# intelligent-machine-learning/tfplus

Hardware: AMD Instinct MI355X
Metric: lookups+GroupAdam-applies/sec and HBM GB/s, 1M int64 ids x dim32 (higher is better)
Workload: dtype f32; 1 GPU; configs[1]: 50M-key KvVariable x dim32 per GPU, 1000000 ids/batch per GPU Zipf(1.2), lookup + sparse GroupAdam apply; keys=50000000, dim=32, batch=1000000, global_batch=1000000, parallelism=single GPU

## Files before the change

include/kvhip.h:

```cpp
#ifndef KVHIP_H_
#define KVHIP_H_

#include <stdint.h>

#ifdef __cplusplus
extern "C" {
#endif

typedef struct kv_table* kv_handle_t;
typedef void* kv_stream_t;

#define KV_OK 0
#define KV_INVALID_ARGUMENT 3
#define KV_RESOURCE_EXHAUSTED 8
#define KV_FAILED_PRECONDITION 9
#define KV_UNIMPLEMENTED 12
#define KV_INTERNAL 13

#define KV_DT_FLOAT 1
#define KV_DT_INT32 3
#define KV_DT_INT64 9
#define KV_DT_UINT64 23

#define KV_SCATTER_ASSIGN 0
// ... 30 lines not shown
                        float* out, kv_stream_t stream);
int kv_gather_or_insert_pairs(kv_handle_t h, const int64_t* id_count_pairs, int64_t n, float* out,
                              kv_stream_t stream);

typedef uint64_t kv_batch_token_t;
int kv_gather_or_insert_tok(kv_handle_t h, const void* ids, const int32_t* counts, int64_t n,
                            float* out, kv_batch_token_t* token, kv_stream_t stream);

int kv_gather_or_zeros(kv_handle_t h, const void* ids, int64_t n, float* out, kv_stream_t stream);


int kv_apply_group_adam(kv_handle_t var, kv_handle_t m_v_linear, const float* grad, const void* ids,
                        int64_t n, float lr, float beta1_power, float beta2_power, float beta1,
                        float beta2, float epsilon, float l1, float l2, float l21, int version,
                        kv_stream_t stream);
int kv_apply_adagrad(kv_handle_t var, kv_handle_t accum, float lr, const float* grad,
                     const void* ids, int64_t n, int update_slots, kv_stream_t stream);
int kv_apply_sparse_group_ftrl(kv_handle_t var, kv_handle_t accum, kv_handle_t linear,
                               const float* grad, const void* ids, int64_t n, float lr, float l1,
                               float l2, float l21, float l2_shrinkage, float lr_power,
                               kv_stream_t stream);

int kv_apply_group_adam_unique(kv_handle_t var, kv_handle_t m_v_linear, const float* grad, const void* ids, int64_t n,
                               float lr, float beta1_power, float beta2_power, float beta1, float beta2, float epsilon,
                               float l1, float l2, float l21, int version, kv_stream_t stream);
int kv_apply_adagrad_unique(kv_handle_t var, kv_handle_t accum, float lr, const float* grad, const void* ids,
                            int64_t n, int update_slots, kv_stream_t stream);
int kv_apply_sparse_group_ftrl_unique(kv_handle_t var, kv_handle_t accum, kv_handle_t linear, const float* grad,
                                      const void* ids, int64_t n, float lr, float l1, float l2, float l21,
                                      float l2_shrinkage, float lr_power, kv_stream_t stream);

int kv_apply_group_adam_tok(kv_handle_t var, kv_handle_t m_v_linear, const float* grad, const void* ids,
                            int64_t n, float lr, float beta1_power, float beta2_power, float beta1,
                            float beta2, float epsilon, float l1, float l2, float l21, int version,
                            kv_batch_token_t token, kv_stream_t stream);
int kv_apply_adagrad_tok(kv_handle_t var, kv_handle_t accum, float lr, const float* grad, const void* ids,
                         int64_t n, int update_slots, kv_batch_token_t token, kv_stream_t stream);
int kv_apply_sparse_group_ftrl_tok(kv_handle_t var, kv_handle_t accum, kv_handle_t linear, const float* grad,
                                   const void* ids, int64_t n, float lr, float l1, float l2, float l21,
                                   float l2_shrinkage, float lr_power, kv_batch_token_t token,
                                   kv_stream_t stream);

int kv_attach_slot(kv_handle_t var, kv_handle_t slot, kv_stream_t stream);

#define KV_ORDER_ARRIVAL 0
#define KV_ORDER_FIXED 1
#define KV_ORDER_OCCURRENCE 2
int kv_set_deterministic(kv_handle_t h, int on);

int kv_set_fast_math(kv_handle_t h, int on);

#define KV_STAT_MIRROR_APPLIES 0
#define KV_STAT_MIRROR_EPOCHS 1
int kv_get_stat(kv_handle_t h, int which, int64_t* value);

int kv_prepare_capture(kv_handle_t h, int64_t max_new_ids, kv_stream_t stream);

int kv_dedup_segment_sum(kv_handle_t h, const void* ids, const float* grad, int64_t n,
                         int64_t* uniq_ids, float* summed, int32_t* inverse, int64_t* num_unique,
                         kv_stream_t stream);

int kv_export_count(kv_handle_t h, int first_n, int64_t* counts, kv_stream_t stream);
int kv_export_fill(kv_handle_t h, int first_n, int64_t* keys, float* values, int64_t* blacklist,
                   int64_t* freq_keys, uint32_t* freq_values, kv_stream_t stream);
int kv_set_delta_tracking(kv_handle_t h, int support_delta_export, int support_prediction_delta_export);
int kv_export_delta_count(kv_handle_t h, int first_n, int64_t* counts, kv_stream_t stream);
int kv_export_delta_fill(kv_handle_t h, int first_n, int64_t* keys, float* values, int64_t* blacklist,
                         int64_t* freq_keys, uint32_t* freq_values, int64_t* delete_keys,
                         kv_stream_t stream);
int kv_import(kv_handle_t h, const int64_t* keys, const float* values, int64_t n,
              const int64_t* blacklist, int64_t n_blacklist, const int64_t* freq_keys,
              const uint32_t* freq_values, int64_t n_freq, kv_stream_t stream);

int kv_import_delta(kv_handle_t h, const int64_t* keys, const float* values, int64_t n,
                    const int64_t* blacklist, int64_t n_blacklist, const int64_t* freq_keys,
                    const uint32_t* freq_values, int64_t n_freq, const int64_t* delete_keys,
                    int64_t n_delete, int first_n, kv_stream_t stream);

int kv_insert(kv_handle_t h, const void* ids, const float* values, int64_t n, kv_stream_t stream);
int kv_scatter_update(kv_handle_t h, const void* ids, const float* updates, int64_t n, int op,
                      kv_stream_t stream);

int kv_unique(kv_handle_t h, const void* ids, const int32_t* counts, int64_t n, int64_t* uniq,
              int32_t* uniq_counts, int32_t* inverse, int64_t* num_unique, int64_t* num_unique_dev,
              kv_stream_t stream);

int kv_get_count(kv_handle_t h, const void* ids, int64_t n, int32_t* counts, kv_stream_t stream);
int kv_get_timestamp(kv_handle_t h, const void* ids, int64_t n, uint32_t* days, kv_stream_t stream);
int kv_delete(kv_handle_t h, const void* ids, int64_t n, int64_t* num_deleted, kv_stream_t stream);
int kv_delete_with_timestamp(kv_handle_t h, int threshold, int dry_run, int64_t* delete_keys,
                             int64_t* count, kv_stream_t stream);

int kv_batch_gather_or_zeros(int num_tables, const kv_handle_t* tables, const void* const* ids,
                             const int64_t* ns, float* const* outs, kv_stream_t stream);

int kv_multi_gather_or_insert(int num_tables, const kv_handle_t* tables, const void* const* ids,
                              const int32_t* const* counts, const int64_t* ns, float* const* outs,
                              kv_stream_t stream);
int kv_multi_apply_group_adam(int num_tables, const kv_handle_t* vars, const kv_handle_t* slots,
                              const float* const* grads, const void* const* ids, const int64_t* ns,
                              float lr, float beta1_power, float beta2_power, float beta1, float beta2,
                              float epsilon, float l1, float l2, float l21, int version,
                              kv_stream_t stream);
int kv_multi_apply_adagrad(int num_tables, const kv_handle_t* vars, const kv_handle_t* accums, float lr,
                           const float* const* grads, const void* const* ids, const int64_t* ns,
                           int update_slots, kv_stream_t stream);
// ... 155 lines not shown
```

tfplus_amd/csrc/kv_apply.hip:

```cpp
#include <hip/hip_runtime.h>

#include <type_traits>

#include "kv_host.h"

using namespace kvhip_internal;

namespace {

static bool claim_slot(kv_table* v, kv_table* sl, hipStream_t s) {
  if (v->slot_uid == sl->uid && v->slot_gen == sl->gen) return true;
  if (v->slot_uid != 0 && v->slot_uid != sl->uid) return false;
  if (v->slot_uid == sl->uid)
    launch_clear_hints(v, s);
  v->slot_uid = sl->uid;
  v->slot_gen = sl->gen;
  return true;
}

static void wrap_uniq_serial(kv_table* v, hipStream_t s) {
  if (v->uniq_serial < 65535u) return;
  launch_clear_stamps(v, s);
  v->uniq_serial = 0;
}
// ... 55 lines not shown
  }
  {
    std::vector<kv_table*> u(all);
    std::sort(u.begin(), u.end());
    if (std::adjacent_find(u.begin(), u.end()) != u.end())
      return fail(KV_INVALID_ARGUMENT, "batched op: a table is listed twice (var or slot)");
  }
  const int device = vars[0]->device;
  DeviceGuard dg(device);
  hipStream_t s = (hipStream_t)stream;
  MultiLock lock(all);
  auto keep = [&](const kv_table* tb) -> unsigned {
    unsigned k = KEEP_NONE;
    if (!two_slots(OPT))
      for (int i = 0; i < num_tables; ++i) k |= (vars[i] == tb ? KEEP_VAR : KEEP_NONE) | (slots0[i] == tb ? KEEP_SLOT : KEEP_NONE);
    return k;
  };
  if (unique && fused_ok(D) && !stream_is_capturing(s)) {
    long long nmax = 0;
    if ((rc = lock.enter(s, keep))) return rc;
    for (int i = 0; i < num_tables; ++i) {
      if ((rc = ensure_capacity(vars[i], ns[i], s)) || (rc = ensure_capacity(slots0[i], ns[i], s)) ||
          (slots1 && (rc = ensure_capacity(slots1[i], ns[i], s))))
        return rc;
      nmax = std::max<long long>(nmax, ns[i]);
    }
    if (nmax == 0) return KV_OK;
    Staged<MultiDesc> hd(device, 1, num_tables);
    if (hd.rc) return hd.rc;
    for (int i = 0; i < num_tables; ++i) {
      kv_table* v = vars[i];
      wrap_uniq_serial(v, s);
      MultiDesc& d = hd[i];
      opt_part_args(d.a, v, slots0[i], slots1 ? slots1[i] : nullptr, a, grads[i], ns[i], s);
      if ((rc = mirror_decide(v, slots0[i], d.a, !two_slots(OPT), s))) return rc;
      d.a.uniq_serial = ns[i] > 0 ? ++v->uniq_serial : 0u;
      d.ids = ids[i];
      d.n = ns[i];
    }
    const MultiDesc* md;
    if ((rc = hd.upload(s, &md))) return rc;
    const int ids32 = vars[0]->key_dtype == KV_DT_INT32 ? 1 : 0;
    ProfScope ps(vars[0], KV_PROF_APPLY_UNIQUE, s);
    rc = launch_uapply<OPT>(hd[0].a, nullptr, ids32, nmax, s, md, num_tables);
    if (rc) return fail(rc, "batched unique apply: no kernel for dim %d", D);
    HIP_TRY(hipGetLastError());
    return KV_OK;
  }
  const bool fz = fused_ok(D);
  bool reuse = tokens != nullptr && fz;
  bool pa_reuse = reuse;
  for (int i = 0; i < num_tables && reuse; ++i)
    if (ns[i] > 0) {
      const bool held = tokens[i] != 0 && tokens[i] == vars[i]->batch_serial && ns[i] == vars[i]->batch_n && vars[i]->fused_index;
      if (!held) reuse = false;
      if (!held || !vars[i]->part_pending) pa_reuse = false;
    }
  if (!reuse) pa_reuse = false;
  for (kv_table* tb : lock.ts) {
    bool taken = false;
    if (pa_reuse)
      for (int i = 0; i < num_tables; ++i) taken = taken || (vars[i] == tb && ns[i] > 0);
    if ((rc = enter_op(tb, s, keep(tb), !taken))) return rc;
  }
  long long nmax = 0;
  if (require_reuse && !reuse)
    return fail(KV_FAILED_PRECONDITION, "batched sharded apply: another op used a table since this batch's lookup");
  for (int i = 0; i < num_tables; ++i) {
    if (!reuse) vars[i]->batch_serial = 0;
    if (!reuse && (rc = ensure_capacity(vars[i], ns[i], s))) return rc;
    if ((rc = ensure_capacity(slots0[i], ns[i], s))) return rc;
    if (slots1 && (rc = ensure_capacity(slots1[i], ns[i], s))) return rc;
    if ((rc = ensure_workspace(vars[i], std::max<long long>(ns[i], 1), true, s))) return rc;
    nmax = std::max<long long>(nmax, ns[i]);
  }
  if (nmax == 0) return KV_OK;
  Staged<MultiDesc> hd(device, 1, num_tables);
  if (hd.rc) return hd.rc;
  WsDev wmax{};
  for (int i = 0; i < num_tables; ++i) {
    MultiDesc& d = hd[i];
    d.w = ws_view(vars[i], std::max<long long>(ns[i], 1), selfs ? &selfs[i] : nullptr);
    if (fz) { d.a.epart = d.w.epart; use_partitions(d.w, fused_default_P(std::max<long long>(ns[i], 1))); }
    opt_part_args(d.a, vars[i], slots0[i], slots1 ? slots1[i] : nullptr, a, grads[i], ns[i], s);
    d.a.det = vars[i]->deterministic ? 1 : 0;
    if ((rc = mirror_decide(vars[i], slots0[i], d.a, fz && !two_slots(OPT), s))) return rc;
    d.ids = ids[i];
    d.n = ns[i];
    if (ns[i] == 0) d.w.ntiles = 0;
    if (reuse && ns[i] > 0 && vars[i]->index_P) use_partitions(d.w, vars[i]->index_P);
    d.a.day_lk = d.a.day;
    if (pa_reuse && ns[i] > 0) {
      PartArgs pend;
      take_pending_part(vars[i], &pend);
      d.a.day_lk = pend.day; d.a.count_once = pend.count_once;
    }
    widen(wmax, d.w);
  }
  const MultiDesc* md;
  if ((rc = hd.upload(s, &md))) return rc;
  if (fz) {
    int pa_mode = pa_reuse ? PA_LOOKUP : PA_NONE;
    if (!reuse) {
      for (int i = 0; i < num_tables; ++i) vars[i]->fused_index = true;
      launch_ltile(vars[0], hd[0].a.tv, wmax, nullptr, nullptr, nmax, nullptr, s, -1, md, num_tables, false);
      pa_mode = PA_APPLYIDX;
      for (int i = 0; i < num_tables; ++i)
        if (ns[i] > 0) { vars[i]->batch_serial = ++g_serial; vars[i]->batch_n = ns[i]; vars[i]->index_P = hd[i].w.P; }
    }
    if ((rc = launch_tsum(hd[0].a.tv, wmax, nullptr, s, md, num_tables)))
      return fail(rc, "tile sums: no kernel for dim %d", D);
    rc = launch_papply<OPT>(wmax, hd[0].a, pa_mode, s, md, num_tables);
    if (rc) return fail(rc, "partition + apply pass: no kernel for dim %d", D);
    HIP_TRY(hipGetLastError());
    return KV_OK;
  }
  for (int i = 0; i < num_tables; ++i) vars[i]->fused_index = false;
  launch_tile<false>(vars[0], wmax, nullptr, nullptr, nmax, s, -1, md, num_tables, wmax.ntiles);
  launch_part_keys<MODE_APPLYIDX>(wmax, hd[0].a, s, md, num_tables);
  launch_order(hd[0].a.tv, wmax, nmax, s, md, num_tables);
  if ((rc = launch_apply<MODE_APPLY, OPT>(vars[0], wmax, hd[0].a, nmax, s, md, num_tables))) return rc;
  HIP_TRY(hipGetLastError());
  return KV_OK;
}

template <int OPT>
static int apply_common(kv_table* v, kv_table* s0, kv_table* s1, const float* grad, const void* ids, int64_t n,
                        const OptArgs& a, kv_batch_token_t token, hipStream_t s, bool unique, const SelfSegment* self) {
  const long long nmax = fused_tab(v) ? FUSED_MAX_N : (1ll << 21);
  if (n < 0 || n > nmax)
    return fail(n < 0 ? KV_INVALID_ARGUMENT : KV_UNIMPLEMENTED,
                "indices: %lld ids in one optimizer call (limit %lld for this embedding dim; split the batch)", (long long)n, nmax);
  if (n > 0 && (!grad || !ids)) return fail(KV_INVALID_ARGUMENT, "grad / indices pointer is null");
  if (!dim_supported(v->dim))
    return fail(KV_UNIMPLEMENTED, "embedding dim %d not supported by the fused kernels", v->dim);
  int rc;
  if (unique && fused_ok(v->dim) && !stream_is_capturing(s)) {
    if ((rc = ensure_capacity(v, n, s)) || (rc = ensure_capacity(s0, n, s)) || (s1 && (rc = ensure_capacity(s1, n, s)))) return rc;
    wrap_uniq_serial(v, s);
    PartArgs pa{};
    opt_part_args(pa, v, s0, s1, a, grad, n, s);
    if ((rc = mirror_decide(v, s0, pa, !two_slots(OPT), s))) return rc;
    pa.uniq_serial = ++v->uniq_serial;
    ProfScope ps(v, KV_PROF_APPLY_UNIQUE, s);
    rc = launch_uapply<OPT>(pa, ids, v->key_dtype == KV_DT_INT32 ? 1 : 0, n, s);
    if (rc) return fail(rc, "unique apply: no kernel for dim %d", v->dim);
    HIP_TRY(hipGetLastError());
    return KV_OK;
  }
  const bool reuse = token != 0 && token == v->batch_serial && n == v->batch_n;
  const bool pa_route = fused_tab(v);
  int pa_mode = -1;
  PartArgs pend{};
  const void* tile_ids = nullptr;
  if (v->part_pending) {
    if (reuse && pa_route && v->fused_index) {
      take_pending_part(v, &pend);
      pa_mode = PA_LOOKUP;
    } else if ((rc = flush_part(v, s))) {
      return rc;
    }
  }
  if (!reuse && (rc = ensure_capacity(v, n, s))) return rc;
  if ((rc = ensure_capacity(s0, n, s))) return rc;
  if (s1 && (rc = ensure_capacity(s1, n, s))) return rc;
  if ((rc = ensure_workspace(v, n, true, s))) return rc;
  WsDev wd = ws_view(v, n, self);
  PartArgs pa{};
  opt_part_args(pa, v, s0, s1, a, grad, n, s);
  pa.det = det_mode(v);
  pa.day_lk = pa.day;
  if (pa_mode == PA_LOOKUP) { pa.day_lk = pend.day; pa.count_once = pend.count_once; }
  if (!reuse) {
    v->batch_serial = 0;
    if (pa_route) {
      v->fused_index = true;
      choose_partitions(v, wd, n);
      tile_ids = ids;
      pa_mode = PA_APPLYIDX;
    } else {
      index_pass<MODE_APPLYIDX>(v, wd, pa, ids, nullptr, n, -1, nullptr, s);
    }
    v->batch_serial = ++g_serial;
    v->batch_n = n;
  } else if (pa_mode < 0 && v->fused_index) {
    pa_mode = PA_NONE;
  }
  if (v->fused_index && reuse && v->index_P) use_partitions(wd, v->index_P);
  if ((rc = mirror_decide(v, s0, pa, v->fused_index && !two_slots(OPT), s))) return rc;
  if (v->fused_index) rc = fused_apply<OPT>(v, wd, pa, n, s, pa_mode, tile_ids);
  else rc = launch_apply<MODE_APPLY, OPT>(v, wd, pa, n, s);
  if (rc) return rc;
  HIP_TRY(hipGetLastError());
  return KV_OK;
}


static int check_hp(float lr, float l1, float l2, float l21, float lr_power, float l2s) {
  if (!(lr > 0.f)) return fail(KV_INVALID_ARGUMENT, "lr is not a positive scalar: %g", lr);
  if (!(l1 >= 0.f)) return fail(KV_INVALID_ARGUMENT, "l1 regularization strength is not a non-negative scalar: %g", l1);
  if (!(l2 >= 0.f)) return fail(KV_INVALID_ARGUMENT, "l2 regularization strength is not a non-negative scalar: %g", l2);
  if (!(l21 >= 0.f)) return fail(KV_INVALID_ARGUMENT, "l21 regularization strength is not a non-negative scalar: %g", l21);
  if (!(lr_power <= 0.f)) return fail(KV_INVALID_ARGUMENT, "lr_power is not a non-positive scalar: %g", lr_power);
  if (!(l2s >= 0.f)) return fail(KV_INVALID_ARGUMENT, "l2 shrinkage regularization strength is not a non-negative scalar: %g", l2s);
  return KV_OK;
}

static OptCall group_adam_call(int version, float lr, float b1p, float b2p, float b1, float b2, float eps, float l1, float l2,
                               float l21) {
  OptCall c;
  if (version != 3 && version != 4) {
    c.status = fail(KV_INVALID_ARGUMENT, "GroupAdam version %d: 3 or 4", version);
    return c;
  }
  c.opt = version == 4 ? OPT_ADAM_V4 : OPT_ADAM_V3;
  c.slot_mult = 3;
  if ((c.status = check_hp(lr, l1, l2, l21, 0.f, 0.f))) return c;
  OptArgs& a = c.a;
  a.lr = lr; a.b1p = b1p; a.b2p = b2p; a.b1 = b1; a.b2 = b2; a.eps = eps;
  if (version == 4) {
    a.l1 = l1 * lr; a.l2 = l2 * lr; a.l21 = l21 * lr;
    a.alpha = lr * std::sqrt(1.f - b2p) / (1.f - b1p);
  } else {
    a.l1 = l1; a.l2 = l2; a.l21 = l21;
    a.alpha = std::sqrt(1.f - b2p) / (1.f - b1p);
  }
  return c;
}
static OptCall adagrad_call(float lr, int update_slots) {
  OptCall c;
  c.opt = OPT_ADAGRAD;
  c.a.lr = lr; c.a.update_slots = update_slots;
  return c;
}
static OptCall sparse_group_ftrl_call(float lr, float l1, float l2, float l21, float l2s, float lr_power) {
  OptCall c;
  c.opt = OPT_FTRL;
  if ((c.status = check_hp(lr, l1, l2, l21, lr_power, l2s))) return c;
  c.a.lr = lr; c.a.l1 = l1; c.a.l2 = l2; c.a.l21 = l21; c.a.l2s = l2s; c.a.lr_power = lr_power;
  return c;
}
// ... 280 lines not shown
```

tfplus_amd/csrc/kv_device.h:

```cpp
#pragma once

constexpr long long EMPTY_KEY = (long long)0x8000000000000000ULL;
constexpr unsigned FLAG_BLACK = 1u;
constexpr unsigned FLAG_UNDER = 2u;
constexpr unsigned FLAG_DIRTY = 4u;
constexpr float CUTOFF = 1.0e-20f;
constexpr unsigned FLAG_FREE = 8u;
constexpr unsigned ROW_TOMB = 0xFFFFFFFFu;
constexpr unsigned ROW_FILTERED = 0x80000000u;
constexpr unsigned ROW_MASK = 0x7FFFFFFFu;
constexpr unsigned HEAD_BIT = 0x80000000u;
constexpr unsigned BASE_MASK = 0x3FFFFFFFu;
constexpr int RANK_SHIFT = 21;
constexpr unsigned SLOT_MASK = (1u << RANK_SHIFT) - 1u;
constexpr int LCOLD = 16;
constexpr int HC = 128;
constexpr unsigned EP_TAG = 0x40000000u;
constexpr unsigned NEW_BIT = 0x80000000u;
constexpr unsigned HINT_NEW = 0xFFFFFFFFu;
constexpr int HC2 = 512;

constexpr int TB = 256;
#ifndef KV_TBT
#define KV_TBT 512
#endif
constexpr int TBT = KV_TBT;
constexpr int IPT = 4;
constexpr int TILE = TBT * IPT;
constexpr int LS = 2 * TILE;
constexpr int MAX_P = 2048;
constexpr int MAX_CHUNKS = 32768;

#ifdef KV_STAMPS
#define KV_STAMP(slot) do { if (threadIdx.x == 0) w.dbg[(size_t)blockIdx.x * 16 + (slot)] = wall_clock64(); } while (0)
#define KV_STAMPP(slot) do { if (threadIdx.x == 0) w.dbg[(size_t)(blockIdx.x + 4096) * 16 + (slot)] = wall_clock64(); } while (0)
#define KV_STAMP_HW(slot) do { if (threadIdx.x == 0) w.dbg[(size_t)blockIdx.x * 16 + (slot)] = \
    ((unsigned long long)__builtin_amdgcn_s_getreg(63508) << 32) | (unsigned)__builtin_amdgcn_s_getreg(63492); } while (0)
#define KV_STAMPPV(slot, v) do { if (threadIdx.x == 0) w.dbg[(size_t)(blockIdx.x + 4096) * 16 + (slot)] = (v); } while (0)
#define KV_STAMPA(slot) do { if (threadIdx.x == 0) w.dbg[(size_t)(blockIdx.x + 8192) * 16 + (slot)] = wall_clock64(); } while (0)
#define KV_STAMPV(slot, v) do { if (threadIdx.x == 0) w.dbg[(size_t)(blockIdx.x + 8192) * 16 + (slot)] = (v); } while (0)
#define KV_STAMPT(slot) do { if (threadIdx.x == 0) w.dbg[(size_t)(blockIdx.x + 2048) * 16 + (slot)] = wall_clock64(); } while (0)
#else
#define KV_STAMP(slot) do { } while (0)
#define KV_STAMPP(slot) do { } while (0)
#define KV_STAMP_HW(slot) do { } while (0)
#define KV_STAMPPV(slot, v) do { } while (0)
#define KV_STAMPA(slot) do { } while (0)
#define KV_STAMPV(slot, v) do { } while (0)
#define KV_STAMPT(slot) do { } while (0)
#endif

template <typename Tag, typename Kernel>
static inline int resident_blocks(Kernel k, int threads, int cap_per_cu, int fallback_per_cu) {
  constexpr int MAXDEV = 64;
  static int cache[MAXDEV];
  int dev = 0;
  hipGetDevice(&dev);
  const bool slot = dev >= 0 && dev < MAXDEV;
  if (slot) { const int c = __atomic_load_n(&cache[dev], __ATOMIC_RELAXED); if (c > 0) return c; }
  int nb = 0, cus = 0;
  hipDeviceGetAttribute(&cus, hipDeviceAttributeMultiprocessorCount, dev);
  if (hipOccupancyMaxActiveBlocksPerMultiprocessor(&nb, k, threads, 0) != hipSuccess || nb < 1) nb = fallback_per_cu;
  if (nb > cap_per_cu) nb = cap_per_cu;
  const int r = nb * (cus > 0 ? cus : 256);
  if (slot) __atomic_store_n(&cache[dev], r, __ATOMIC_RELAXED);
  return r;
}

__device__ __forceinline__ unsigned long long mix64(unsigned long long x) {
  x ^= x >> 33; x *= 0xff51afd7ed558ccdULL;
  x ^= x >> 33; x *= 0xc4ceb9fe1a85ec53ULL;
  x ^= x >> 33;
  return x;
}
__device__ __forceinline__ unsigned long long pick64(unsigned long long x) {
  x ^= x >> 30; x *= 0xbf58476d1ce4e5b9ULL;
  x ^= x >> 27; x *= 0x94d049bb133111ebULL;
  x ^= x >> 31;
  return x;
}

__device__ __forceinline__ float* row_ptr(const TableDev& t, unsigned r) {
  if (t.single || (r >> t.chunk_bits) == 0) return t.c0.rows + (size_t)r * t.dim;
// ... 599 lines not shown
```

tfplus_amd/csrc/kv_fused.h:

```cpp
#pragma once

__device__ __forceinline__ unsigned tile_insert(const TableDev& t, long long key) {
  Entry* slot;
  unsigned long long stored;
  unsigned long long p = 0;
  const bool sentinel = key == EMPTY_KEY;
  if (sentinel) { slot = &t.entries[t.mask + 1]; stored = 0ull; }
  else { stored = (unsigned long long)key; p = mix64((unsigned long long)key) & t.mask; slot = &t.entries[p]; }
  for (;;) {
    const Entry e = load_entry(slot);
    if ((unsigned long long)e.key == stored && !(sentinel && e.key == EMPTY_KEY)) {
      if (e.row == ROW_TOMB) {
        if (atomicCAS(&slot->row, ROW_TOMB, 0u) == ROW_TOMB) break;
        return NEW_BIT;
      }
      if (e.row == 0u || e.hint == HINT_NEW) return NEW_BIT | e.row;
      return e.row;
    }
    if (e.key == EMPTY_KEY) {
      const unsigned long long old = atomicCAS(reinterpret_cast<unsigned long long*>(&slot->key),
                                               (unsigned long long)EMPTY_KEY, stored);
      if (old == (unsigned long long)EMPTY_KEY) break;
      if (old == stored) return NEW_BIT;
      if (sentinel) continue;
    } else if (sentinel) {
      return NEW_BIT;
    }
    if (!sentinel) { p = (p + 1) & t.mask; slot = &t.entries[p]; }
  }
  unsigned r = 0;
  bool have = false;
  if (t.free_rows) {
    const int f = atomicSub(reinterpret_cast<int*>(&t.counters[2]), 1);
    if (f > 0) { r = t.free_rows[f - 1]; have = true; }
    else atomicAdd(reinterpret_cast<int*>(&t.counters[2]), 1);
  }
  if (!have) {
    r = atomicAdd(&t.counters[0], 1u);
    if (r >= t.max_rows) { raise_error(t, 1u); return NEW_BIT; }
  }
  *reinterpret_cast<uint2*>(&slot->row) = make_uint2(r, HINT_NEW);
  return NEW_BIT | r;
}

struct LtSmem {
  long long* lkeys;
  unsigned* lrow;
  unsigned* escan;
  unsigned* lcnt;
  unsigned short* lpos;
  unsigned* mr;
  unsigned short* lrun;
  unsigned* hist;
  unsigned* wtot;
};
constexpr size_t LT_KEYS_BYTES = (size_t)(LS + 1) * 8 + 64;
static_assert(LT_KEYS_BYTES >= (((size_t)(LS + 1) * 4 + 15) & ~(size_t)15) + (((size_t)(TILE + 1) * 4 + 15) & ~(size_t)15) + (size_t)TILE * 4, "aliases fit");

__host__ __device__ inline size_t ltile_smem_bytes() {
  size_t b = LT_KEYS_BYTES + 16;
  b += (size_t)(LS + 1) * 4 + 16;
  b += (size_t)(LS + 1) * 2 + 16;
  b += (size_t)(TILE + 1) * 2 + 16;
  b += (size_t)(MAX_P + 1) * 4 + 16;
  b += 64;
  return b;
}
__device__ __forceinline__ LtSmem carve_ltile(char* base) {
  LtSmem s;
  auto take = [&](size_t bytes) { char* p = base; base += (bytes + 15) & ~(size_t)15; return p; };
  char* k0 = take(LT_KEYS_BYTES);
  s.lkeys = reinterpret_cast<long long*>(k0);
  s.lrow = reinterpret_cast<unsigned*>(k0);
  s.escan = reinterpret_cast<unsigned*>(k0 + (((size_t)(LS + 1) * 4 + 15) & ~(size_t)15));
  s.mr = reinterpret_cast<unsigned*>(k0 + (((size_t)(LS + 1) * 4 + 15) & ~(size_t)15) + (((size_t)(TILE + 1) * 4 + 15) & ~(size_t)15));
  s.lcnt = reinterpret_cast<unsigned*>(take((size_t)(LS + 1) * 4));
  s.lpos = reinterpret_cast<unsigned short*>(take((size_t)(LS + 1) * 2));
  s.lrun = reinterpret_cast<unsigned short*>(take((size_t)(TILE + 1) * 2));
  s.hist = reinterpret_cast<unsigned*>(take((size_t)(MAX_P + 1) * 4));
  s.wtot = reinterpret_cast<unsigned*>(take(64));
  return s;
}

constexpr unsigned ES_POS = 0xFFFu, ES_NSH = 12;
static_assert(TILE <= (1 << 11), "mrow: the tile-local position is an 11-bit field");
static_assert(TILE / 2 <= (1 << 10), "mrow: the entry's epart row is a 10-bit field (an entry in mrow has >= 2 rows)");
static_assert(TILE <= (int)ES_POS && TILE / 2 < (1 << (23 - ES_NSH)), "escan: rows and entry numbers of a tile fit their fields");
static_assert(TILE <= 65535, "toff / hist / mcount pack per-tile counts into 16-bit halves");
constexpr int LT_TOUCH_MAXENT = TILE / 2;

template <typename IdT, int VQ, bool GATHER, bool NOTABLE = false>
__device__ __forceinline__ void ltile_body(const TableDev& t, const WsDev& w, const IdT* __restrict__ ids,
                                           const int* __restrict__ counts, long long n, int det,
                                           float* __restrict__ out) {
  extern __shared__ __attribute__((aligned(16))) char smem_raw[];
  LtSmem sm = carve_ltile(smem_raw);
  __shared__ unsigned lsent;

  const int tid = threadIdx.x;
  const unsigned tile = blockIdx.x;
  const long long base = (long long)tile * TILE;
  const unsigned P = w.P;
  constexpr bool PAIRS = std::is_same<IdT, IdCount>::value;
  const bool has_counts = PAIRS || counts != nullptr;
  KV_STAMP(0);
  KV_STAMP_HW(10);

  long long kreg[IPT];
  unsigned creg[IPT];
  unsigned there = 0;
#pragma unroll
  for (int k = 0; k < IPT; ++k) {
    const long long i = base + (long long)k * TBT + tid;
    if (i < n) there |= 1u << k;
    const long long ic = i < n ? i : n - 1;
    if constexpr (PAIRS) kreg[k] = load_id(((unsigned)ic - w.self_lo < w.self_len) ? static_cast<const IdT*>(w.ids_self) : ids, (size_t)ic);
    else kreg[k] = load_id(ids, (size_t)ic);
    creg[k] = 1;
  }
  if constexpr (PAIRS) {
#pragma unroll
    for (int k = 0; k < IPT; ++k) {
      const long long i = base + (long long)k * TBT + tid;
      const long long ic = i < n ? i : n - 1;
      const long long ci = (((unsigned)ic - w.self_lo < w.self_len) ? static_cast<const IdT*>(w.ids_self) : ids)[ic].count;
      creg[k] = (unsigned)(unsigned short)(ci < 65535 ? ci : 65535);
    }
  } else if (counts != nullptr) {
#pragma unroll
    for (int k = 0; k < IPT; ++k) {
      const long long i = base + (long long)k * TBT + tid;
      const int ci = counts[i < n ? i : n - 1];
      creg[k] = (unsigned)(unsigned short)(ci < 65535 ? ci : 65535);
    }
  }
  unsigned long long pp[IPT];
  Entry en[IPT];
  auto issue_probes = [&](unsigned mask) {
#pragma unroll
    for (int k = 0; k < IPT; ++k) {
      pp[k] = 0ull;
      en[k] = Entry{0, 0u, 0u};
      if constexpr (!NOTABLE) {
        pp[k] = ((mask >> k) & 1u) ? home_of(t, kreg[k], mix64((unsigned long long)kreg[k])) : 0ull;
        en[k] = load_entry(&t.entries[pp[k]]);
      }
    }
  };
  unsigned rr[IPT], hn[IPT];
  float pf = 0.f;
#pragma unroll
  for (int k = 0; k < IPT; ++k) { rr[k] = 0u; hn[k] = 0u; }
  auto resolve_probes = [&](unsigned mask) {
    if constexpr (!NOTABLE) {
#pragma unroll
      for (int k = 0; k < IPT; ++k) {
        if (!((mask >> k) & 1u)) continue;
        unsigned hint = 0;
        unsigned r = table_find_from(t, kreg[k], pp[k], en[k], &hint);
        if (__builtin_expect(r == 0u, 0)) { r = NEW_BIT; hint = 0; }
        else if (__builtin_expect(hint == HINT_NEW, 0)) { r |= NEW_BIT; hint = 0; }
        rr[k] = r; hn[k] = hint;
      }
    }
  };
  for (int s = tid; s <= LS; s += TBT) { sm.lkeys[s] = EMPTY_KEY; sm.lcnt[s] = 0; }
  for (unsigned p = tid; p <= P; p += TBT) sm.hist[p] = 0;
  if (tid == 0) lsent = 0;
  if (tile == 0 && tid == 0 && t.err_host)
    __hip_atomic_store(t.err_host + 1, w.ctr[5], __ATOMIC_RELAXED, __HIP_MEMORY_SCOPE_SYSTEM);
  lds_barrier();
  if (tile == 0 && tid < 8) w.ctr[tid] = 0;
  if constexpr (PAIRS) {
#pragma unroll
    for (int k = 0; k < IPT; ++k) {
      const long long i = base + (long long)k * TBT + tid;
      if (!((there >> k) & 1u)) continue;
      bool ok = creg[k] != 0u;
      if (ok && w.seg_cap) {
        const long long r = i % w.seg_cap;
        const long long ih = i - r;
        ok = r >= 1 && r <= (((unsigned)ih - w.self_lo < w.self_len) ? static_cast<const IdT*>(w.ids_self) : ids)[ih].id;
      }
      if (!ok) there &= ~(1u << k);
    }
  }
  lds_barrier();
  KV_STAMP(7);

  auto output_rows = [&]() {
    if constexpr (GATHER) {
      constexpr int RW = 64 / VQ;
      constexpr int CW = VQ < 8 ? VQ : 8;
      const int lane = tid & 63;
      const int v = lane % VQ, sub = lane / VQ;
      const int D4 = t.dim >> 2;
      const bool vlive = v < D4;
      const int vv = vlive ? v : 0;
      auto copy_rows = [&](auto single_tag) {
        constexpr bool SINGLE = decltype(single_tag)::value;
        const float4* rows0 = reinterpret_cast<const float4*>(t.c0.rows);
        constexpr int SPK = VQ / CW;
        constexpr int NP = IPT * SPK;
        auto issue = [&](int pc, float4 (&val)[CW]) {
          const int k = pc / SPK, j0 = (pc % SPK) * CW;
#pragma unroll
          for (int j = 0; j < CW; ++j) {
            const unsigned rj = __shfl(rr[k], (j0 + j) * RW + sub) & ROW_MASK;
            if constexpr (SINGLE) val[j] = rows0[(size_t)rj * D4 + vv];
            else val[j] = reinterpret_cast<const float4*>(row_ptr(t, rj))[vv];
          }
        };
        auto flush = [&](int pc, float4 (&val)[CW]) {
          const int k = pc / SPK, j0 = (pc % SPK) * CW;
          const long long r0 = base + (long long)k * TBT + (tid & ~63);
          if (__builtin_expect(__ballot((rr[k] & NEW_BIT) != 0u) != 0ull, 0)) {
#pragma unroll
            for (int j = 0; j < CW; ++j) {
              const unsigned rj = __shfl(rr[k], (j0 + j) * RW + sub);
              const long long kj = __shfl(kreg[k], (j0 + j) * RW + sub);
              if (rj & NEW_BIT) {
                const unsigned long long h = pick64((unsigned long long)kj ^ (t.seed * 0x9E3779B97F4A7C15ULL));
                const float4 a = reinterpret_cast<const float4*>(t.init_table + (size_t)((unsigned)h % t.init_rows) * t.dim)[vv];
                const float4 b = reinterpret_cast<const float4*>(t.init_table + (size_t)((unsigned)(h >> 32) % t.init_rows) * t.dim)[vv];
                val[j] = make_float4((a.x + b.x) * 0.5f, (a.y + b.y) * 0.5f, (a.z + b.z) * 0.5f, (a.w + b.w) * 0.5f);
// ... 29 lines not shown
          }
        } else {
#pragma unroll
          for (int pc = 0; pc < NP; ++pc) {
            issue(pc, va);
            flush(pc, va);
            asm volatile("" ::: "memory");
          }
        }
      };
      if (single_chunk(t)) copy_rows(std::true_type{}); else copy_rows(std::false_type{});
    }
  };
  unsigned tslot[IPT], myrank[IPT];
  unsigned win = 0;
#pragma unroll
  for (int k = 0; k < IPT; ++k) {
    tslot[k] = 0xFFFFFFFFu;
    myrank[k] = 0;
    if ((there >> k) & 1u) {
      const long long key = kreg[k];
      unsigned h;
      if (key == EMPTY_KEY) {
        h = LS;
        if (atomicCAS(&lsent, 0u, 1u) == 0u) win |= 1u << k;
      } else {
        h = (unsigned)(mix64((unsigned long long)key) >> 40) & (LS - 1);
        for (;;) {
          const unsigned long long old = atomicCAS(reinterpret_cast<unsigned long long*>(&sm.lkeys[h]),
                                                   (unsigned long long)EMPTY_KEY, (unsigned long long)key);
          if (old == (unsigned long long)EMPTY_KEY) { win |= 1u << k; break; }
          if (old == (unsigned long long)key) break;
          h = (h + 1) & (LS - 1);
        }
      }
      myrank[k] = atomicAdd(&sm.lcnt[h], 1u);
      tslot[k] = h;
    }
  }
  KV_STAMP(8);
  issue_probes(win);
  if constexpr (NOTABLE) {
    if (w.zero_counts) {
#pragma unroll
      for (int k = 0; k < IPT; ++k) {
        const long long i = base + (long long)k * TBT + tid;
        if (i < n) w.zero_counts[i] = 0;
      }
    }
  }
  KV_STAMP(9);
  lds_barrier();
  KV_STAMP(1);

  unsigned wcnt[IPT], wp[IPT], wr[IPT];
#pragma unroll
  for (int k = 0; k < IPT; ++k) {
    wcnt[k] = 0; wp[k] = 0; wr[k] = 0;
    if ((win >> k) & 1u) {
      wcnt[k] = sm.lcnt[tslot[k]];
      wp[k] = part_of(kreg[k], w.pshift);
      wr[k] = atomicAdd(&sm.hist[wp[k]], 1u | (wcnt[k] << 16)) & 0xFFFFu;
    }
  }
  lds_barrier();
  {
    const unsigned per = (P + TBT - 1) / TBT;
    const unsigned p0 = tid * per, p1 = min(p0 + per, P);
    unsigned sum = 0;
    for (unsigned p = p0; p < p1; ++p) sum += sm.hist[p];
    unsigned tot;
    unsigned run = block_excl_scan<TBT / 64, true>(sum, sm.wtot, &tot);
    for (unsigned p = p0; p < p1; ++p) { const unsigned c = sm.hist[p]; sm.hist[p] = run; run += c; }
    if (tid == 0) sm.hist[P] = tot;
  }
  lds_barrier();
  const unsigned nent = sm.hist[P] & 0xFFFFu;
  for (unsigned p = tid; p <= P; p += TBT) w.toff[(size_t)tile * (P + 1) + p] = sm.hist[p];
  unsigned wpos[IPT];
#pragma unroll
  for (int k = 0; k < IPT; ++k) {
    wpos[k] = 0xFFFFFFFFu;
    if ((win >> k) & 1u) {
      wpos[k] = (sm.hist[wp[k]] & 0xFFFFu) + wr[k];
      w.ent_key[(size_t)tile * TILE + wpos[k]] = kreg[k];
    }
  }
  if (det) {
    __syncthreads();
    unsigned npos[IPT];
#pragma unroll
    for (int k = 0; k < IPT; ++k) {
      npos[k] = 0xFFFFFFFFu;
      if (wpos[k] == 0xFFFFFFFFu) continue;
      const unsigned p0 = sm.hist[wp[k]] & 0xFFFFu, p1 = sm.hist[wp[k] + 1u] & 0xFFFFu;
      unsigned less = 0;
      for (unsigned j = p0; j < p1; ++j) less += w.ent_key[(size_t)tile * TILE + j] < kreg[k] ? 1u : 0u;
      npos[k] = p0 + less;
    }
    __syncthreads();
#pragma unroll
    for (int k = 0; k < IPT; ++k) {
      if (npos[k] == 0xFFFFFFFFu) continue;
      wpos[k] = npos[k];
      w.ent_key[(size_t)tile * TILE + wpos[k]] = kreg[k];
    }
  }
#pragma unroll
  for (int k = 0; k < IPT; ++k) {
    if (wpos[k] == 0xFFFFFFFFu) continue;
    sm.lpos[tslot[k]] = (unsigned short)wpos[k];
    if (!has_counts) w.ent_a[(size_t)tile * TILE + wpos[k]] = wcnt[k] | (wcnt[k] << 16);
    sm.escan[wpos[k]] = wcnt[k] > 1u ? (wcnt[k] | (1u << ES_NSH)) : 0u;
  }
  lds_barrier();
  KV_STAMP(2);

  {
    constexpr unsigned PER = (TILE + 1 + TBT - 1) / TBT;
    const unsigned e0 = tid * PER, e1 = min(e0 + PER, nent);
    unsigned sum = 0;
    for (unsigned e = e0; e < e1; ++e) sum += sm.escan[e];
    unsigned tot;
    unsigned run = block_excl_scan<TBT / 64, true>(sum, sm.wtot, &tot);
    for (unsigned e = e0; e < e1; ++e) { const unsigned c = sm.escan[e]; sm.escan[e] = run; run += c; }
    if (tid == 0) w.mcount[tile] = (tot & ES_POS) | ((tot >> ES_NSH) << 16);
  }
  resolve_probes(win);
#pragma unroll
  for (int k = 0; k < IPT; ++k) {
    if (wpos[k] == 0xFFFFFFFFu) continue;
    unsigned r = rr[k];
    if constexpr (!NOTABLE) {
      if (__builtin_expect((r & ROW_MASK) == 0u, 0)) r = tile_insert(t, kreg[k]);
    }
    const size_t e = (size_t)tile * TILE + wpos[k];
    sm.lrow[tslot[k]] = r;
    w.ent_b[e] = r;
    w.ent_base[e] = hn[k];
    if (GATHER && nent <= (unsigned)LT_TOUCH_MAXENT && (r & ROW_MASK) != 0u && !(r & NEW_BIT))
      pf += *reinterpret_cast<const volatile float*>(row_ptr(t, r & ROW_MASK));
  }
  lds_barrier();
  KV_STAMP(3);
  if (w.pos_ent) {
#pragma unroll
    for (int k = 0; k < IPT; ++k) {
      const long long i = base + (long long)k * TBT + tid;
      if (i < n) w.pos_ent[i] = tslot[k] != 0xFFFFFFFFu ? sm.lpos[tslot[k]] : (unsigned short)0xFFFFu;
    }
  }
#pragma unroll
  for (int k = 0; k < IPT; ++k) {
    if (wpos[k] == 0xFFFFFFFFu) continue;
    const unsigned pre = sm.escan[wpos[k]];
    w.ent_rec[(size_t)tile * TILE + wpos[k]] = wcnt[k] > 1u ? (EP_TAG | (tile * (unsigned)(TILE / 2) + (pre >> ES_NSH)))
                                                            : (unsigned)base + (unsigned)(k * TBT + tid);
  }
  if (det) {
    unsigned short* run = sm.lrun;
    for (int e = tid; e <= TILE; e += TBT) run[e] = 0;
    lds_barrier();
    const int lane = tid & 63, wave = tid >> 6;
#pragma unroll
    for (int k = 0; k < IPT; ++k) {
      const bool valid = tslot[k] != 0xFFFFFFFFu;
      const unsigned e = valid ? (unsigned)sm.lpos[tslot[k]] : 0u;
      unsigned long long mask = __ballot(valid);
#pragma unroll
      for (int b = 0; b < 11; ++b) {
        const bool bit = (e >> b) & 1u;
        const unsigned long long bal = __ballot(bit);
        mask &= bit ? bal : ~bal;
      }
      const unsigned rw = (unsigned)__popcll(mask & ((1ull << lane) - 1ull));
      const unsigned cnt = (unsigned)__popcll(mask);
      unsigned before = 0;
      for (int wv = 0; wv < TBT / 64; ++wv) {
        if (wave == wv && valid) {
          before = run[e];
          if (rw == 0u) run[e] = (unsigned short)(before + cnt);
        }
        lds_barrier();
      }
      myrank[k] = valid ? before + rw : 0u;
    }
  }
#pragma unroll
  for (int k = 0; k < IPT; ++k) {
    if (tslot[k] == 0xFFFFFFFFu || sm.lcnt[tslot[k]] <= 1u) continue;
    const unsigned pre = sm.escan[sm.lpos[tslot[k]]];
    sm.mr[(pre & ES_POS) + myrank[k]] = (unsigned)(k * TBT + tid) | ((pre >> ES_NSH) << 11) | (myrank[k] == 0u ? 0x80000000u : 0u);
  }
  if (has_counts) {
    lds_barrier();
    for (unsigned e = tid; e <= (unsigned)TILE; e += TBT) sm.hist[e] = 0;
    lds_barrier();
#pragma unroll
    for (int k = 0; k < IPT; ++k)
      if (tslot[k] != 0xFFFFFFFFu) atomicAdd(&sm.hist[sm.lpos[tslot[k]]], creg[k]);
    lds_barrier();
#pragma unroll
    for (int k = 0; k < IPT; ++k) {
      if (wpos[k] == 0xFFFFFFFFu) continue;
      const unsigned f = sm.hist[wpos[k]];
      w.ent_a[(size_t)tile * TILE + wpos[k]] = wcnt[k] | ((f > 65535u ? 65535u : f) << 16);
    }
  }
  lds_barrier();
  {
    unsigned* dst = w.mrow + (size_t)tile * TILE;
    for (int j = tid; j < TILE; j += TBT) dst[j] = sm.mr[j];
  }
  KV_STAMP(4);
  if constexpr (GATHER) {
#pragma unroll
    for (int k = 0; k < IPT; ++k) rr[k] = tslot[k] != 0xFFFFFFFFu ? sm.lrow[tslot[k]] : 0u;
    if (__builtin_expect(pf == 1.2345678e-38f, 0)) sm.wtot[0] = 1u;
    output_rows();
  }
  KV_STAMP(5);
}

template <typename IdT, int VQ, bool GATHER, bool NOTABLE = false>
__global__ void __launch_bounds__(TBT, 4) k_ltile(TableDev t, WsDev w, const IdT* __restrict__ ids,
                                              const int* __restrict__ counts, long long n, int det, float* __restrict__ out) {
  ltile_body<IdT, VQ, GATHER, NOTABLE>(t, w, ids, counts, n, det, out);
}

template <int T, int NW>
__device__ __forceinline__ unsigned seg_directory_t(const WsDev& w, unsigned p, unsigned short* tpre,
                                                    unsigned short* tstart, unsigned* wtot, unsigned* pbase) {
  const unsigned NT = w.ntiles;
  unsigned run0 = 0, pb = 0;
  for (unsigned tb = 0; tb < NT; tb += T) {
    const unsigned t = tb + threadIdx.x;
    unsigned len = 0, s0 = 0;
    if (t < NT) {
      const unsigned* c0 = w.toff + (size_t)t * (w.P + 1) + p;
      const unsigned a = c0[0], b = c0[1];
      s0 = a & 0xFFFFu;
      len = (b & 0xFFFFu) - s0;
      tstart[t] = (unsigned short)s0;
    }
    unsigned tot;
    const unsigned ex = block_excl_scan<NW>(len, wtot, &tot);
    unsigned tot2;
    block_excl_scan<NW>(s0, wtot, &tot2);
    if (t < NT) tpre[t] = (unsigned short)min(run0 + ex, 65535u);
    run0 += tot;
    pb += tot2;
  }
  __syncthreads();
  *pbase = pb;
  return run0;
}
__device__ __forceinline__ void part2_body(const WsDev& w, const PartArgs& a) {
  constexpr int HSK = 1024;
  constexpr int UCAPK = HSK - TBK;
  constexpr int EB = 8;
  __shared__ long long hkey[HSK + 1];
  __shared__ unsigned hval[HSK + 1];
  __shared__ unsigned hrow[HSK + 1];
  __shared__ unsigned short lnew[UCAPK + 8];
  __shared__ unsigned short ulist[UCAPK + 8];
  __shared__ unsigned lnu, lsent, lnnew, lkeys;
  __shared__ unsigned wtot[8];
  extern __shared__ __attribute__((aligned(16))) char smem_raw[];
  unsigned short* tpre = reinterpret_cast<unsigned short*>(smem_raw);
  unsigned short* tstart = tpre + w.ntiles;

  const int tid = threadIdx.x;
  const unsigned p = xcd_partition(blockIdx.x, w.P);
  const unsigned NT = w.ntiles;
  const int D = a.tv.dim;
  KV_STAMPP(0);
  unsigned pbase;
  const unsigned E = seg_directory_t<TBK, TBK / 64>(w, p, tpre, tstart, wtot, &pbase);
  if (E == 0) return;
  __shared__ unsigned stkR[24], stkr[24];
  __shared__ int sp;
  if (tid == 0) { stkR[0] = 1; stkr[0] = 0; sp = 1; lkeys = 0; }
  __syncthreads();
  if (E > 65535u) {
    if (tid == 0) raise_error(a.tv, 2u);
    return;
  }
  while (sp > 0) {
    const unsigned R = stkR[sp - 1], round = stkr[sp - 1];
    __syncthreads();
    if (tid == 0) --sp;
    for (int s = tid; s <= HSK; s += TBK) { hkey[s] = EMPTY_KEY; hval[s] = 0; hrow[s] = 0; }
    if (tid == 0) { lnu = 0; lsent = 0; lnnew = 0; }
    __syncthreads();
    for (unsigned x0 = 0; x0 < E; x0 += EB * TBK) {
      unsigned ge[EB];
      long long key[EB];
      unsigned ea[EB], rw[EB];
#pragma unroll
      for (int k = 0; k < EB; ++k) {
        const unsigned x = x0 + k * TBK + tid;
        ge[k] = x < E ? (unsigned)seg_entry(tpre, tstart, NT, x) : 0xFFFFFFFFu;
      }
#pragma unroll
      for (int k = 0; k < EB; ++k) {
        key[k] = 0; ea[k] = 0; rw[k] = 0;
        if (ge[k] != 0xFFFFFFFFu) { key[k] = w.ent_key[ge[k]]; ea[k] = w.ent_a[ge[k]]; rw[k] = w.ent_b[ge[k]]; }
      }
#pragma unroll
      for (int k = 0; k < EB; ++k) {
        if (ge[k] == 0xFFFFFFFFu || !in_round(key[k], R, round)) continue;
        if (lnu >= (unsigned)UCAPK) continue;
        bool first;
        const unsigned h = lds_key_slot<HSK>(hkey, &lsent, key[k], true, &first);
        if (first) {
          const unsigned u = atomicAdd(&lnu, 1u);
          if (u < (unsigned)UCAPK) ulist[u] = (unsigned short)h;
        }
        atomicAdd(&hval[h], ea[k] >> 16);
        atomicMax(&hrow[h], rw[k]);
      }
    }
    __syncthreads();
    if (lnu >= (unsigned)UCAPK) {
      __syncthreads();
      if (tid == 0) {
        if (sp + 2 <= 24) {
          stkR[sp] = 2 * R; stkr[sp] = round; ++sp;
          stkR[sp] = 2 * R; stkr[sp] = round + R; ++sp;
        } else {
          raise_error(a.tv, 2u);
        }
      }
      __syncthreads();
      continue;
    }
    KV_STAMPP(1);
    const unsigned nu = lnu;
    if (tid == 0) lkeys += nu;

    constexpr int PERU = (UCAPK + TBK - 1) / TBK;
    {
      unsigned sl[PERU], r[PERU];
      bool isnew[PERU];
      uint2 m[PERU];
#pragma unroll
      for (int k = 0; k < PERU; ++k) {
// ... 331 lines not shown
```

tfplus_amd/csrc/kv_host.h:

```cpp
#pragma once

#include <algorithm>
#include <atomic>
#include <cmath>
#include <cstdarg>
#include <cstdint>
#include <cstdio>
#include <cstring>
#include <mutex>
#include <string>
#include <type_traits>
#include <vector>

#include "../../include/kvhip.h"
#include "kv_launch.h"

namespace __attribute__((visibility("hidden"))) kvhip_internal {

int fail(int code, const char* fmt, ...);

#define HIP_TRY(expr)                                                                         \
  do {                                                                                        \
    hipError_t _e = (expr);                                                                   \
    if (_e != hipSuccess)                                                                     \
      return fail(_e == hipErrorOutOfMemory ? KV_RESOURCE_EXHAUSTED : KV_INTERNAL,            \
                  "%s failed: %s (%s:%d)", #expr, hipGetErrorString(_e), __FILE__, __LINE__); \
  } while (0)

struct Workspace {
  long long cap_n = 0;
  unsigned capP = 0;
  long long* ent_key = nullptr;
  unsigned* ent_a = nullptr;
  unsigned* ent_b = nullptr;
  unsigned* ent_base = nullptr;
  unsigned* ent_rec = nullptr;
  unsigned* toff = nullptr;
  unsigned* slot_rank = nullptr;
  unsigned* order = nullptr;
  uint4* coldlist = nullptr;
  uint4* hotlist = nullptr;
  uint4* litem = nullptr;
  uint4* items = nullptr;
  uint4* pmeta = nullptr;
  float* hpart = nullptr;
  long long hpart_elems = 0;
  unsigned* ctr = nullptr;
  unsigned* mcount = nullptr;
  unsigned short* pos_ent = nullptr;
  long long pos_cap = 0;
  float* epart = nullptr;
  long long epart_elems = 0;
  long long* scat_keys = nullptr;
  float* scat_sum = nullptr;
  long long scat_cap = 0;
  unsigned* seg_off = nullptr;
  long long seg_cap = 0;
  unsigned long long* dbg = nullptr;
};

}

using namespace kvhip_internal;

struct kv_table {
  uint64_t op_serial = 1, export_serial = 0, delta_serial = 0, expire_serial = 0;
  int device = 0;
  int key_dtype = KV_DT_INT64;
  int dim = 0;
  unsigned enter_threshold = 0;
  unsigned long long seed = 0;
  int fixed_day = -1;
  Entry* entries = nullptr;
  unsigned long long cap = 0;
  int chunk_bits = 16;
  std::vector<Chunk> chunks;
  Chunk* d_chunks = nullptr;
  unsigned* d_counters = nullptr;
  unsigned* free_rows = nullptr;
  unsigned long long free_cap = 0;
  long long free_known = 0;
  unsigned long long idx_ub = 0;
  unsigned long long idx_base = 0, bump_base = 1, pushes_since = 0;
  long long free_base = 0;
  unsigned long long rows_cap = 0;
  unsigned long long rows_ub = 1;
  float* init_table = nullptr;
  long long init_rows = 0;
  bool initialized = false;
  bool init_placeholder = false;
  Workspace ws;
  uint64_t batch_serial = 0;
  long long batch_n = 0;
  bool fused_index = false;
  long long batch_n_prev = 0;
  unsigned index_P = 0;
  bool part_pending = false;
  unsigned char pend_wd[sizeof(WsDev)], pend_pa[sizeof(PartArgs)];
  long long stat_mirror_applies = 0;
  std::atomic<long long> stat_mirror_epochs{0};
  TableDev mview_var{}, mview_slot{};
  kv_table* mirror_slot = nullptr;
  std::atomic<unsigned> mirror_epoch{1};
  std::atomic<bool> mirror_dirty{false};
  kv_table* mirror_var = nullptr;
  bool mirror_banned = false;
  bool mirror_shared = false;
  unsigned uniq_serial = 0;
  bool deterministic = false;
  bool occurrence_order = false;
  std::atomic<int> shard_refs{0};
  bool fast_math = false;
  uint64_t uid = 0;
  uint64_t slot_uid = 0;
  uint64_t slot_gen = 0;
  uint64_t gen = 0;
  unsigned* err_host = nullptr;
  unsigned* cnt_host = nullptr;
  hipStream_t last_stream = nullptr;
  bool has_last = false;
  hipEvent_t last_done = nullptr;
  bool track_delta = false, track_pred = false;
  std::vector<long long> del_train, del_pred;
  unsigned long long* d_stat = nullptr;
  std::mutex mu;
  unsigned* route_hist = nullptr;
  size_t route_hist_cap = 0;
  bool prof = false;
  unsigned prof_mask = 0xFFFFFFFFu;
  std::vector<hipEvent_t> ev;
  std::vector<int> ev_kind;
  size_t ev_used = 0;
  int prof_every = 1;
  unsigned prof_seq[KV_PROF_KINDS] = {};
};

namespace __attribute__((visibility("hidden"))) kvhip_internal {

inline unsigned long long pow2ceil(unsigned long long x) {
  unsigned long long p = 1;
  while (p < x) p <<= 1;
  return p;
}

inline int ilog2(unsigned long long x) {
  int l = 0;
  while ((1ull << l) < x) ++l;
  return l;
}
// ... 124 lines not shown
                  const MultiDesc* md = nullptr, int ntab = 0);
void launch_ltile(kv_table* t, const TableDev& td, const WsDev& wd, const void* ids, const int* counts, long long n, float* out,
                  hipStream_t s, int ids_kind = -1, const MultiDesc* md = nullptr, int ntab = 0, bool multi_rows = false);
void launch_part2(const WsDev& wd, const PartArgs& pa, hipStream_t s, const MultiDesc* md = nullptr, int ntab = 0);
int launch_occ_sum(const WsDev& wd, const PartArgs& pa, int fop, long long nmax, hipStream_t s);
void launch_fill_entries(kv_table* t, hipStream_t s);
void launch_clear_hints(kv_table* v, hipStream_t s);
void launch_clear_stamps(kv_table* v, hipStream_t s);
void launch_link_hints(kv_table* v, kv_table* sl, unsigned nrows, hipStream_t s);
void launch_ltile_notable(kv_table* t, const TableDev& td, const WsDev& wd, const void* ids, long long n, hipStream_t s,
                          const int* counts = nullptr, bool int32_ids = false);
void launch_ltile_multi_notable(const WsDev& wmax, int ntab, const MultiDesc* md, hipStream_t s);

enum : unsigned {
  KEEP_NONE = 0u,
  KEEP_VAR = 1u,
  KEEP_SLOT = 2u,
};

int hand_over(kv_table* t, hipStream_t s, unsigned keep = KEEP_NONE, bool settle = true, bool mutates = true);
int enter_op(kv_table* t, hipStream_t s, unsigned keep = KEEP_NONE, bool settle = true, bool mutates = true);
int join_side(kv_table* t, hipStream_t s);
int settle_pending(kv_table* t);
int stats(kv_handle_t t, hipStream_t s, unsigned long long out[2], unsigned* nrows_out);

void set_pending_part(kv_table* t, const WsDev& wd, const PartArgs& pa);
void take_pending_part(kv_table* t, PartArgs* lookup);
int flush_part(kv_table* t, hipStream_t s);
int mirror_decide(kv_table* v, kv_table* s0, PartArgs& pa, bool lean, hipStream_t s);

struct MultiLock {
  std::vector<kv_table*> ts;
  explicit MultiLock(std::initializer_list<kv_table*> l) : MultiLock(std::vector<kv_table*>(l)) {}
  explicit MultiLock(std::vector<kv_table*> l) : ts(std::move(l)) {
    std::sort(ts.begin(), ts.end());
    ts.erase(std::unique(ts.begin(), ts.end()), ts.end());
    for (auto* t : ts) t->mu.lock();
  }
  ~MultiLock() { for (auto it = ts.rbegin(); it != ts.rend(); ++it) (*it)->mu.unlock(); }
  template <class Keep>
  int enter(hipStream_t s, Keep keep, kv_table* later = nullptr) {
    int rc;
    for (auto* t : ts)
      if ((rc = enter_op(t, s, keep(t), t != later))) return rc;
    return KV_OK;
  }
  int enter(hipStream_t s) { return enter(s, [](const kv_table*) { return (unsigned)KEEP_NONE; }); }
};

void retire_stream(hipStream_t dead);

extern std::atomic<uint64_t> g_serial;
void choose_partitions(kv_table* t, WsDev& wd, long long n);
template <int MODE>
void index_pass(kv_table* t, const WsDev& wd, const PartArgs& pa, const void* ids, const int* counts, long long n,
                int ids_kind, float* out, hipStream_t s, bool file_order = true);
int fused_lookup_pass(kv_table* t, WsDev& wd, const PartArgs& pa, const void* ids, const int* counts, long long n,
                      int ids_kind, float* out, hipStream_t s, bool defer_part);
template <int MODE, int OPT>
int launch_apply(kv_table* prof_t, const WsDev& wd, const PartArgs& pa, long long nmax, hipStream_t s,
                 const MultiDesc* md = nullptr, int ntab = 0, bool skip_fin = false) {
  const int D = pa.tv.dim;
  constexpr int gmax = 2048;
  const unsigned grid = (unsigned)std::max<long long>(1, std::min<long long>(gmax, (nmax / 2 + chunk_cap(nmax)) / 4 + 1));
  const unsigned gfin = (unsigned)std::max<long long>(1, std::min<long long>(256, nmax / 4096 + 1));
  auto launch = [&](unsigned nchunks, int span) {
    if constexpr (MODE == MODE_DEDUP) return launch_dedup_fold(wd, pa, s, md, ntab, nchunks, span);
    else return launch_sorted_apply<OPT>(wd, pa, s, md, ntab, nchunks, span);
  };
  int rc;
  if (pa.det == 2 && !md) {
    const int fop = MODE == MODE_APPLY ? KV_SCATTER_ADD : pa.fold_op;
    if ((rc = launch_occ_sum(wd, pa, fop, nmax, s))) return rc;
  }
  {
    ProfScope ps(prof_t, KV_PROF_APPLY_SORTED, s);
    rc = launch(grid, 0);
  }
  if (rc == KV_OK && !skip_fin) {
    ProfScope ps(prof_t, KV_PROF_APPLY_SPAN, s);
    rc = launch(gfin, 1);
  }
  if (rc == KV_UNIMPLEMENTED)
    return md ? fail(KV_UNIMPLEMENTED, "batched launch: embedding dim %d (multiples of 4 only)", D)
              : fail(KV_UNIMPLEMENTED, "embedding dim %d not supported by the fused kernels "
                     "(multiples of 4 up to 1024, any dim up to 256)", D);
  return KV_OK;
}

struct StageSlot {
  char* host = nullptr;
  char* dev = nullptr;
  size_t cap = 0;
  hipEvent_t consumed = nullptr;
};
struct BatchStage {
  std::mutex mu;
  StageSlot slot[4];
  unsigned cursor = 0;
};
extern BatchStage g_stage[64][2];
int stage_take(BatchStage& st, size_t bytes, StageSlot** out);
template <class Desc>
class Staged {
  BatchStage& st;
  StageSlot* sl = nullptr;
  const size_t bytes;
  hipStream_t s = nullptr;
  bool launched = false;
 public:
  int rc;
// ... 47 lines not shown
```

tfplus_amd/csrc/kv_ops.hip:

```cpp
#include <hip/hip_runtime.h>

#include <iterator>

#include "kv_host.h"

using namespace kvhip_internal;

namespace {

#include "kv_device.h"
#include "kv_op_kernels.h"

static int record_deleted(kv_table* t, const void* ids, int64_t n, bool int32_ids, hipStream_t s) {
  if (!t->track_delta || n <= 0) return KV_OK;
  const size_t base = t->del_train.size();
  t->del_train.resize(base + (size_t)n);
  if (int32_ids) {
    std::vector<int> tmp((size_t)n);
    HIP_TRY(hipMemcpyAsync(tmp.data(), ids, (size_t)n * sizeof(int), hipMemcpyDeviceToHost, s));
    HIP_TRY(hipStreamSynchronize(s));
    for (int64_t i = 0; i < n; ++i) t->del_train[base + (size_t)i] = tmp[(size_t)i];
  } else {
    HIP_TRY(hipMemcpyAsync(t->del_train.data() + base, ids, (size_t)n * sizeof(long long), hipMemcpyDeviceToHost, s));
    HIP_TRY(hipStreamSynchronize(s));
// ... 97 lines not shown

static int dedup_locked(kv_table* t, const void* ids, const float* grad, int64_t n, int64_t* uniq,
                        float* summed, int32_t* inverse, int64_t* num_unique, int fold_op, hipStream_t s) {
  int rc;
  if ((rc = ensure_workspace(t, n, true, s))) return rc;
  WsDev wd = ws_view(t, n);
  t->batch_serial = 0;
  PartArgs pa = self_part_args(t, n);
  pa.grad = grad;
  pa.out_keys = (long long*)uniq;
  pa.out_sum = summed;
  pa.fold_op = fold_op;
  pa.dd_number = 1;
  if ((rc = segment_sums(t, wd, pa, ids, n, t->key_dtype == KV_DT_INT32, true, "per-id sums", s))) return rc;
  if (inverse && t->fused_index) k_inverse_e<<<nblocks(n, TB, 2048), TB, 0, s>>>(t->ws.pos_ent, wd.ent_b, n, inverse);
  else if (inverse) k_dedup_inverse<<<nblocks(n, TB, 2048), TB, 0, s>>>(wd, n, inverse);
  unsigned U = 0;
  if ((rc = read_count(t, wd.ctr, s, &U))) return rc;
  *num_unique = U;
  return KV_OK;
}

static int ensure_free_list(kv_table* t, hipStream_t s) {
  if (t->free_cap >= t->rows_cap) return KV_OK;
  unsigned* nf = nullptr;
  HIP_TRY(hipStreamSynchronize(s));
  HIP_TRY(hipMalloc(&nf, (size_t)t->rows_cap * sizeof(unsigned)));
  if (t->free_rows) {
    HIP_TRY(hipMemcpy(nf, t->free_rows, (size_t)t->free_cap * sizeof(unsigned), hipMemcpyDeviceToDevice));
    hipFree(t->free_rows);
  }
  t->free_rows = nf;
  t->free_cap = t->rows_cap;
  return KV_OK;
}

static int after_release(kv_table* t, hipStream_t s, unsigned long long* released) {
  unsigned c[3];
  unsigned long long n = 0;
  HIP_TRY(hipMemcpyAsync(&n, t->d_stat, sizeof n, hipMemcpyDeviceToHost, s));
  HIP_TRY(hipMemcpyAsync(c, t->d_counters, sizeof c, hipMemcpyDeviceToHost, s));
  HIP_TRY(hipStreamSynchronize(s));
  t->pushes_since += n;
  t->free_known = std::max(0, (int)c[2]);
  t->rows_ub = c[0];
  *released = n;
  return KV_OK;
}

static int delete_locked(kv_table* t, const void* ids, int64_t n, int64_t* num_deleted, hipStream_t s) {
  int rc;
  if ((rc = enter_op(t, s))) return rc;
  t->batch_serial = 0;
  if ((rc = ensure_free_list(t, s))) return rc;
  HIP_TRY(hipMemsetAsync(t->d_stat, 0, 4 * sizeof(unsigned long long), s));
  with_id_type(t->key_dtype == KV_DT_INT32, [&](auto id) {
    using IDT = decltype(id);
    k_delete<IDT><<<nblocks(n, TB, 4096), TB, 0, s>>>(dev_view(t), (const IDT*)ids, n, t->free_rows, t->d_stat);
  });
  HIP_TRY(hipGetLastError());
  unsigned long long rel = 0;
  if ((rc = after_release(t, s, &rel))) return rc;
  if (num_deleted) *num_deleted = (int64_t)rel;
  return KV_OK;
}

static int count_or_ts(kv_handle_t t, const void* ids, int64_t n, int what, uint32_t* out, kv_stream_t stream) {
  int rc;
  if ((rc = check_table(t))) return rc;
  if (n < 0 || (n > 0 && (!ids || !out))) return fail(KV_INVALID_ARGUMENT, "indices / output pointer is null");
  if ((rc = require_initialized(t))) return rc;
  if (n == 0) return KV_OK;
  TableOp op(t, stream);
  if ((rc = join_side(t, op.s))) return rc;
  with_id_type(t->key_dtype == KV_DT_INT32, [&](auto id) {
    using IDT = decltype(id);
    k_get_count_ts<IDT><<<nblocks(n, TB, 4096), TB, 0, op.s>>>(dev_view(t), (const IDT*)ids, n, what, today(t), out);
  });
  HIP_TRY(hipGetLastError());
  return KV_OK;
}

static int scatter_like(kv_handle_t t, const void* ids, const float* vals, int64_t n, int op,
                        int is_insert, int mark, const unsigned* fvals, hipStream_t s) {
  int rc;
  if (n == 0) return KV_OK;
  if (n < 0 || !ids || (!vals && mark < 0)) return fail(KV_INVALID_ARGUMENT, "bad arguments");
  if (!is_insert && mark < 0 && (rc = require_initialized(t))) return rc;
  const long long CH = 1ll << 21;
  const size_t idsz = t->key_dtype == KV_DT_INT32 ? 4 : 8;
  for (long long off = 0; off < n; off += CH) {
    const long long m = std::min(CH, (long long)n - off);
    if ((rc = ensure_capacity(t, m, s))) return rc;
    if ((rc = ensure_workspace(t, m, false, s))) return rc;
    const WsDev wd = ws_view(t, m);
    PartArgs pa = self_part_args(t, m);
    if (!t->initialized) {
      pa.tv.init_table = t->chunks[0].rows;
      pa.tv.init_rows = 1;
      pa.ts0 = pa.tv; pa.ts1 = pa.tv;
    }
    pa.grad = vals ? vals + (size_t)off * t->dim : nullptr;
    pa.scatter_op = op; pa.is_insert = is_insert;
    pa.mark_what = mark; pa.fvals = fvals ? fvals + off : nullptr;
    t->batch_serial = 0;
    launch_tile<true>(t, wd, (const char*)ids + (size_t)off * idsz, nullptr, m, s);
// ... 38 lines not shown
  }
  return KV_OK;
}

}

namespace __attribute__((visibility("hidden"))) kvhip_internal {
int multi_common(int num_tables, const kv_handle_t* tables, const void* const* ids, const int64_t* ns) {
  int rc;
  if ((rc = check_same_shape(num_tables, tables, "tables"))) return rc;
  if (!ids || !ns) return fail(KV_INVALID_ARGUMENT, "null argument array");
  for (int i = 0; i < num_tables; ++i) {
    if (tables[i]->dim != tables[0]->dim || tables[i]->key_dtype != tables[0]->key_dtype)
      return fail(KV_INVALID_ARGUMENT, "batched op: tables must share dim and key dtype (group them by shape)");
    if (tables[i]->occurrence_order)
      return fail(KV_UNIMPLEMENTED, "batched op: a table in occurrence-order mode (kv_set_deterministic(h, 2)) takes the per-table ops");
    if (ns[i] < 0 || ns[i] > (fused_tab(tables[0]) ? FUSED_MAX_N : (1ll << 21)))
      return fail(KV_INVALID_ARGUMENT, "indices: bad length %lld", (long long)ns[i]);
    if (ns[i] > 0 && !ids[i]) return fail(KV_INVALID_ARGUMENT, "indices pointer is null");
    if ((rc = require_initialized(tables[i]))) return rc;
    for (int j = 0; j < i; ++j)
      if (tables[j] == tables[i]) return fail(KV_INVALID_ARGUMENT, "batched op: table listed twice");
  }
  return KV_OK;
}

int gather_or_insert_impl(kv_handle_t t, const void* ids, const int32_t* counts, int64_t n, float* out,
                          kv_stream_t stream, int pairs, kv_batch_token_t* token, unsigned seg_cap,
                          const SelfSegment* self) {
  int rc;
  if ((rc = check_table(t))) return rc;
  if (n == 0) return KV_OK;
  if (n < 0 || n > (1ll << 30)) return fail(KV_INVALID_ARGUMENT, "indices: bad length %lld", (long long)n);
  if (!ids || !out) return fail(KV_INVALID_ARGUMENT, "indices / output pointer is null");
  if ((rc = require_initialized(t))) return rc;
  TableOp tab(t, stream);
  const hipStream_t s = tab.s;
  if ((rc = enter_op(t, s, KEEP_VAR))) return rc;
  const long long CHK = fused_tab(t) ? FUSED_MAX_N : (1ll << 21);
  const size_t idsz = pairs ? 16 : (t->key_dtype == KV_DT_INT32 ? 4 : 8);
  t->batch_serial = 0;
  for (long long off = 0; off < n; off += CHK) {
    const long long m = std::min(CHK, (long long)n - off);
    const void* idp = (const char*)ids + (size_t)off * idsz;
    const int32_t* cp = counts ? counts + off : nullptr;
    float* op = out + (size_t)off * t->dim;
    if ((rc = ensure_capacity(t, m, s))) return rc;
    if ((rc = ensure_workspace(t, m, false, s))) return rc;
    WsDev wd = ws_view(t, m, self);
    wd.seg_cap = seg_cap;
    PartArgs pa = self_part_args(t, m);
    pa.day = today(t);
    const bool defer_part = token != nullptr && n <= CHK;
    if (fused_tab(t)) { if ((rc = fused_lookup_pass(t, wd, pa, idp, cp, m, pairs ? 2 : -1, op, s, defer_part))) return rc; }
    else index_pass<MODE_LOOKUP>(t, wd, pa, idp, cp, m, pairs ? 2 : -1, op, s, token != nullptr && n <= CHK);
  }
  HIP_TRY(hipGetLastError());
  if (token && n <= CHK) {
    t->batch_serial = ++g_serial;
    t->batch_n = n;
    if (token) *token = t->batch_serial;
  }
  return KV_OK;
}

int multi_lookup_impl(int num_tables, const kv_handle_t* tables, const void* const* ids,
                      const int32_t* const* counts, const int64_t* ns, float* const* outs,
                      kv_batch_token_t* tokens, kv_stream_t stream, int ids_kind, const unsigned* seg_caps,
                      const SelfSegment* selfs) {
  int rc;
  if (tokens && num_tables > 0) std::memset(tokens, 0, (size_t)num_tables * sizeof(kv_batch_token_t));
  if ((rc = multi_common(num_tables, tables, ids, ns))) return rc;
  if (!outs) return fail(KV_INVALID_ARGUMENT, "null argument array");
  const int device = tables[0]->device;
  DeviceGuard dg(device);
  hipStream_t s = (hipStream_t)stream;
  MultiLock lock(std::vector<kv_table*>(tables, tables + num_tables));
  if ((rc = lock.enter(s, [](const kv_table*) { return (unsigned)KEEP_VAR; }))) return rc;
  long long nmax = 0;
  for (int i = 0; i < num_tables; ++i) {
    tables[i]->batch_serial = 0;
    if (ns[i] > 0 && !outs[i]) return fail(KV_INVALID_ARGUMENT, "output pointer is null");
    if ((rc = ensure_capacity(tables[i], ns[i], s))) return rc;
    if ((rc = ensure_workspace(tables[i], std::max<long long>(ns[i], 1), false, s))) return rc;
    nmax = std::max<long long>(nmax, ns[i]);
  }
  if (nmax == 0) return KV_OK;
  Staged<MultiDesc> hd(device, 1, num_tables);
  if (hd.rc) return hd.rc;
  WsDev wmax{};
  for (int i = 0; i < num_tables; ++i) {
    MultiDesc& d = hd[i];
    d.w = ws_view(tables[i], std::max<long long>(ns[i], 1), selfs ? &selfs[i] : nullptr);
    if (seg_caps) d.w.seg_cap = seg_caps[i];
    if (fused_tab(tables[i])) use_partitions(d.w, fused_default_P(std::max<long long>(ns[i], 1)));
    d.a = self_part_args(tables[i], ns[i]);
    d.a.day = today(tables[i]);
    d.ids = ids[i];
    d.counts = counts ? counts[i] : nullptr;
    d.out = outs[i];
    d.n = ns[i];
    if (ns[i] == 0) d.w.ntiles = 0;
    widen(wmax, d.w);
  }
  const MultiDesc* md;
  if ((rc = hd.upload(s, &md))) return rc;
  kv_table* t0 = tables[0];
  if (fused_tab(t0)) {
    for (int i = 0; i < num_tables; ++i) tables[i]->fused_index = true;
    launch_ltile(t0, hd[0].a.tv, wmax, nullptr, nullptr, nmax, nullptr, s, ids_kind, md, num_tables, true);
    const bool defer = tokens != nullptr;
    if (!defer) launch_part2(wmax, hd[0].a, s, md, num_tables);
    if (tokens)
      for (int i = 0; i < num_tables; ++i) {
        if (ns[i] <= 0) continue;
        tables[i]->batch_serial = ++g_serial;
        tables[i]->batch_n = ns[i];
        tables[i]->index_P = hd[i].w.P;
        tokens[i] = tables[i]->batch_serial;
        if (defer) set_pending_part(tables[i], hd[i].w, hd[i].a);
      }
  } else {
    for (int i = 0; i < num_tables; ++i) tables[i]->fused_index = false;
    launch_tile<false>(t0, wmax, nullptr, nullptr, nmax, s, -1, md, num_tables, wmax.ntiles);
    launch_part_keys<MODE_LOOKUP>(wmax, hd[0].a, s, md, num_tables);
    launch_gather(hd[0].a.tv, wmax, nullptr, nmax, s, md, num_tables);
  }
  HIP_TRY(hipGetLastError());
  return KV_OK;
}
}

extern "C" {

int kv_size(kv_handle_t t, int64_t* out, kv_stream_t stream) { return read_figure(t, 0, out, stream); }
int kv_sum_freq(kv_handle_t t, int64_t* out, kv_stream_t stream) { return read_figure(t, 1, out, stream); }
int kv_map_size(kv_handle_t t, int64_t* out, kv_stream_t stream) { return read_figure(t, 2, out, stream); }

int kv_get_meta(kv_handle_t t, const int64_t* ids, int64_t n, uint32_t* fw, uint8_t* fl, kv_stream_t stream) {
  int rc;
  if ((rc = check_table(t))) return rc;
  if (n <= 0) return KV_OK;
  TableOp op(t, stream);
  if ((rc = join_side(t, op.s))) return rc;
  k_get_meta<long long><<<nblocks(n, TB), TB, 0, op.s>>>(dev_view(t), (const long long*)ids, n, fw, fl);
  HIP_TRY(hipGetLastError());
  return KV_OK;
}

int kv_gather_or_insert(kv_handle_t t, const void* ids, const int32_t* counts, int64_t n, float* out,
                        kv_stream_t stream) {
  return gather_or_insert_impl(t, ids, counts, n, out, stream, 0, nullptr);
}
int kv_gather_or_insert_tok(kv_handle_t t, const void* ids, const int32_t* counts, int64_t n, float* out,
                            kv_batch_token_t* token, kv_stream_t stream) {
  if (token) *token = 0;
  return gather_or_insert_impl(t, ids, counts, n, out, stream, 0, token);
}
int kv_gather_or_insert_pairs(kv_handle_t t, const int64_t* id_count_pairs, int64_t n, float* out,
                              kv_stream_t stream) {
  if (t && t->key_dtype == KV_DT_INT32) return fail(KV_INVALID_ARGUMENT, "id/count pairs carry int64 ids");
  return gather_or_insert_impl(t, id_count_pairs, nullptr, n, out, stream, 1, nullptr);
// ... 198 lines not shown
  if (n == 0) {
    if (num_unique_dev) HIP_TRY(hipMemsetAsync(num_unique_dev, 0, sizeof(int64_t), (hipStream_t)stream));
    return KV_OK;
  }
  if (n < 0 || !ids || !uniq) return fail(KV_INVALID_ARGUMENT, "bad arguments");
  if (n > FUSED_MAX_N) return fail(KV_UNIMPLEMENTED, "%lld ids in one call (limit 2^23)", (long long)n);
  TableOp op(t, stream);
  const hipStream_t s = op.s;
  if ((rc = enter_op(t, s, KEEP_VAR | KEEP_SLOT))) return rc;
  if ((rc = ensure_workspace(t, n, false, s))) return rc;
  WsDev wd = ws_view(t, n);
  t->batch_serial = 0;
  PartArgs pa = self_part_args(t, n);
  pa.out_keys = (long long*)uniq;
  pa.out_counts = uniq_counts;
  if ((rc = fused_unique_pass(t, wd, pa, ids, counts, n, s))) return rc;
  if (inverse) k_inverse_e<<<nblocks(n, TB, 2048), TB, 0, s>>>(t->ws.pos_ent, wd.ent_b, n, inverse);
  if (num_unique_dev) k_store_count<<<1, 1, 0, s>>>(wd.ctr, (long long*)num_unique_dev);
  HIP_TRY(hipGetLastError());
  if (num_unique) {
    unsigned U = 0;
    if ((rc = read_count(t, wd.ctr, s, &U))) return rc;
    *num_unique = U;
  }
  return KV_OK;
}

int kv_delete(kv_handle_t t, const void* ids, int64_t n, int64_t* num_deleted, kv_stream_t stream) {
  int rc;
  if ((rc = check_table(t))) return rc;
  if (num_deleted) *num_deleted = 0;
  if (n < 0 || (n > 0 && !ids)) return fail(KV_INVALID_ARGUMENT, "indices pointer is null");
  if ((rc = require_initialized(t))) return rc;
  if (n == 0) return KV_OK;
  TableOp op(t, stream);
  if ((rc = record_deleted(t, ids, n, t->key_dtype == KV_DT_INT32, op.s))) return rc;
  return delete_locked(t, ids, n, num_deleted, op.s);
}

int kv_delete_with_timestamp(kv_handle_t t, int threshold, int dry_run, int64_t* out_keys, int64_t* count,
                             kv_stream_t stream) {
  int rc;
  if ((rc = check_table(t))) return rc;
  if (!count || (!dry_run && !out_keys)) return fail(KV_INVALID_ARGUMENT, "count / delete_keys pointer is null");
  if ((rc = require_initialized(t))) return rc;
  TableOp op(t, stream);
  const hipStream_t s = op.s;
  if (!dry_run) {
    if (t->expire_serial != t->op_serial)
      return fail(KV_FAILED_PRECONDITION, "the table was used between the dry run and kv_delete_with_timestamp: the key "
                                          "buffer sized from the count may be too small; count again");
    ++t->op_serial;
    t->batch_serial = 0;
  }
  unsigned nrows = 1;
  if ((rc = stats(t, s, nullptr, &nrows))) return rc;
  if (!dry_run && (rc = ensure_free_list(t, s))) return rc;
  HIP_TRY(hipMemsetAsync(t->d_stat, 0, 4 * sizeof(unsigned long long), s));
  const unsigned thr = (unsigned)(threshold & 0xFFFF);
  k_delete_by_time<<<nblocks(nrows, TB, 4096), TB, 0, s>>>(dev_view(t), nrows, today(t), thr, dry_run ? 0 : 1,
                                                        t->free_rows, t->d_stat, (long long*)out_keys);
  HIP_TRY(hipGetLastError());
  unsigned long long rel = 0;
  if (dry_run) {
    HIP_TRY(hipMemcpyAsync(&rel, t->d_stat, sizeof rel, hipMemcpyDeviceToHost, s));
    HIP_TRY(hipStreamSynchronize(s));
  } else if ((rc = after_release(t, s, &rel))) {
    return rc;
  }
  *count = (int64_t)rel;
  if (dry_run) t->expire_serial = t->op_serial;
  if (!dry_run && (rc = record_deleted(t, out_keys, (int64_t)rel, false, s))) return rc;
  return KV_OK;
}

int kv_get_count(kv_handle_t t, const void* ids, int64_t n, int32_t* counts, kv_stream_t stream) {
  return count_or_ts(t, ids, n, 0, (uint32_t*)counts, stream);
}
int kv_get_timestamp(kv_handle_t t, const void* ids, int64_t n, uint32_t* days, kv_stream_t stream) {
  return count_or_ts(t, ids, n, 1, days, stream);
}

int kv_take_rows(int device, const void* src, const int32_t* index, const int32_t* index_outer, int64_t n,
                 int64_t row_bytes, int scatter, void* out, kv_stream_t stream) {
  if (index_outer && scatter) return fail(KV_INVALID_ARGUMENT, "kv_take_rows: the two-level index is gather only");
  if (n < 0 || row_bytes <= 0 || row_bytes % 4 || (n > 0 && (!src || !index || !out)))
    return fail(KV_INVALID_ARGUMENT, "kv_take_rows: n %lld, row_bytes %lld (a positive multiple of 4)",
                (long long)n, (long long)row_bytes);
  if (n == 0) return KV_OK;
  DeviceGuard dg(device);
  hipStream_t s = (hipStream_t)stream;
  const bool wide = row_bytes % 16 == 0 && ((uintptr_t)src % 16 == 0) && ((uintptr_t)out % 16 == 0);
  const unsigned nu = (unsigned)(row_bytes / (wide ? 16 : 4));
  const int sh = (nu & (nu - 1)) == 0 ? ilog2(nu) : -1;
  const int grid = nblocks(n * nu, TB * 4, 8192);
  if (wide) {
    if (scatter) k_take_rows<float4, 1><<<grid, TB, 0, s>>>((const float4*)src, index, n, nu, sh, (float4*)out);
    else k_take_rows<float4, 0><<<grid, TB, 0, s>>>((const float4*)src, index, n, nu, sh, (float4*)out, index_outer);
  } else {
    if (scatter) k_take_rows<float, 1><<<grid, TB, 0, s>>>((const float*)src, index, n, nu, sh, (float*)out);
    else k_take_rows<float, 0><<<grid, TB, 0, s>>>((const float*)src, index, n, nu, sh, (float*)out, index_outer);
  }
  HIP_TRY(hipGetLastError());
  return KV_OK;
}

// ... 121 lines not shown
    for (long long off = 0; off < n; off += CHK) {
      const long long m = std::min(CHK, (long long)n - off);
      int64_t U = 0;
      if ((rc = dedup_locked(t, (const char*)ids + (size_t)off * idsz, updates + (size_t)off * t->dim, m,
                             (int64_t*)w.scat_keys, w.scat_sum, nullptr, &U, fold, s)))
        return rc;
      if (t->key_dtype == KV_DT_INT32 && U > 0)
        k_narrow_keys<<<1, 1024, 0, s>>>(w.scat_keys, U);
      if ((rc = scatter_like(t, w.scat_keys, w.scat_sum, U, op, 0, -1, nullptr, s))) return rc;
    }
    return KV_OK;
  }
  return scatter_like(t, ids, updates, n, op, 0, -1, nullptr, s);
}

int kv_import_delta(kv_handle_t t, const int64_t* keys, const float* values, int64_t n, const int64_t* blacklist,
                    int64_t n_black, const int64_t* fkeys, const uint32_t* fvals, int64_t n_freq,
                    const int64_t* delete_keys, int64_t n_delete, int first_n, kv_stream_t stream) {
  int rc;
  if ((rc = check_table(t))) return rc;
  TableOp op(t, stream);
  const hipStream_t s = op.s;
  if (t->key_dtype == KV_DT_INT32) return fail(KV_UNIMPLEMENTED, "import with int32 keys");
  if ((rc = enter_op(t, s))) return rc;
  if ((rc = scatter_like(t, keys, values, n, KV_SCATTER_ASSIGN, 3, -1, nullptr, s))) return rc;
  if (n_black > 0) {
    if (first_n > 3) {
      if ((rc = scatter_like(t, blacklist, nullptr, n_black, 0, 1, 0, nullptr, s))) return rc;
    } else if ((rc = delete_locked(t, blacklist, n_black, nullptr, s))) {
      return rc;
    }
  }
  if (n_freq > 0 && (rc = scatter_like(t, fkeys, nullptr, n_freq, 0, 1, 1, fvals, s))) return rc;
  if (n_delete > 0 && (rc = delete_locked(t, delete_keys, n_delete, nullptr, s))) return rc;
  if ((rc = ensure_init_placeholder(t, s))) return rc;
  t->initialized = true;
  HIP_TRY(hipGetLastError());
  return KV_OK;
}

int kv_import(kv_handle_t t, const int64_t* keys, const float* values, int64_t n, const int64_t* blacklist,
              int64_t n_black, const int64_t* fkeys, const uint32_t* fvals, int64_t n_freq,
              kv_stream_t stream) {
  int rc;
  if ((rc = check_table(t))) return rc;
  TableOp op(t, stream);
  const hipStream_t s = op.s;
  if (t->key_dtype == KV_DT_INT32) return fail(KV_UNIMPLEMENTED, "import with int32 keys");
  if ((rc = enter_op(t, s))) return rc;
  HIP_TRY(hipStreamSynchronize(s));
  t->gen += 1;
  t->slot_uid = 0;
  t->batch_serial = 0;
  unsigned init[3] = {1, 0, 0};
  HIP_TRY(hipMemcpy(t->d_counters, init, sizeof init, hipMemcpyHostToDevice));
  launch_fill_entries(t, s);
  t->rows_ub = 1;
  t->idx_ub = t->idx_base = 0; t->bump_base = 1; t->pushes_since = 0; t->free_base = 0; t->free_known = 0;
  t->del_train.clear(); t->del_pred.clear();
  if ((rc = scatter_like(t, keys, values, n, KV_SCATTER_ASSIGN, 2, -1, nullptr, s))) return rc;
  if (n_black > 0 && (rc = scatter_like(t, blacklist, nullptr, n_black, 0, 1, 0, nullptr, s))) return rc;
  if (n_freq > 0 && (rc = scatter_like(t, fkeys, nullptr, n_freq, 0, 1, 1, fvals, s))) return rc;
  if ((rc = ensure_init_placeholder(t, s))) return rc;
  t->initialized = true;
  HIP_TRY(hipGetLastError());
  return KV_OK;
}

}
```

tfplus_amd/csrc/kv_papply.h:

```cpp
#pragma once

#ifndef KV_PA_WAVES
#define KV_PA_WAVES 4
#endif
#ifndef KV_PA_HOTRB
#define KV_PA_HOTRB 8
#endif
template <int TBP> struct PaShape { static constexpr int HSK = TBP >= 512 ? 2048 : 1024, LSRC = TBP >= 512 ? 2048 : 1536; };

template <int OPT, int V, int LPR, int K, int TBP, int FM = -1>
__device__ __forceinline__ void papply_body(const WsDev& w, const PartArgs& a, const int mode_) {
  constexpr bool UQ = FM == PA_UNIQUE, DN = FM == PA_DEDUP_NUM, DD = FM == PA_DEDUP || DN;
  const int mode = FM >= 0 ? (DN ? (int)PA_DEDUP : FM) : (mode_ & 0xFF);
  constexpr int HSK = PaShape<TBP>::HSK;
  constexpr int PA_LSRC = PaShape<TBP>::LSRC;
  constexpr int UCAPK = (HSK - TBP) < 1023 ? (HSK - TBP) : 1023;
  constexpr int EB = 8;
  constexpr int G = 64 / LPR;
  constexpr int RB = (KV_PA_HOTRB / K) > 0 ? (KV_PA_HOTRB / K) : 1;
  constexpr int NW = TBP / 64;
  __shared__ long long hkey[HSK + 1];
  __shared__ unsigned hval[DD ? 1 : HSK + 1];
  __shared__ unsigned hrow[HSK + 1];
  __shared__ unsigned hhint[(UQ || DD) ? 1 : HSK + 1];
  __shared__ unsigned hocc[HSK + 1];
  __shared__ unsigned short hcn[HSK + 1];
  __shared__ unsigned short ulist[UCAPK + 8];
  __shared__ unsigned short kord[UCAPK + 8];
  __shared__ unsigned lsrc[PA_LSRC];
  __shared__ unsigned lnu, lsent, lnext, lkeys, lbase;
  __shared__ unsigned rh[MAXW], rbase[MAXW];
  __shared__ unsigned wtot[8];
  __shared__ unsigned stkR[24], stkr[24];
  __shared__ int sp;
  extern __shared__ __attribute__((aligned(16))) char smem_raw[];
  unsigned short* tpre = reinterpret_cast<unsigned short*>(smem_raw);
  unsigned short* tstart = tpre + w.ntiles;

  const int tid = threadIdx.x;
  const unsigned p = xcd_partition(blockIdx.x, w.P);
  const unsigned NT = w.ntiles;
  const int D = a.tv.dim;
  const unsigned errflag = *reinterpret_cast<volatile unsigned*>(&a.tv.counters[1]);
  KV_STAMPP(0);
  unsigned pbase = 0;
  const unsigned E = seg_directory_t<TBP, NW>(w, p, tpre, tstart, wtot, &pbase);
  KV_STAMPP(5);
  if (E == 0) return;
  if (tid == 0) { sp = 0; lkeys = 0; }
  __syncthreads();
  if (E > 65535u) {
    if (tid == 0) raise_error(a.tv, 2u);
    return;
  }
  const bool in_lds = E <= (unsigned)PA_LSRC;
  unsigned* const gsrc = w.order + pbase;
  auto src_at = [&](unsigned i) -> unsigned {
    return in_lds ? lsrc[i] : __hip_atomic_load(gsrc + i, __ATOMIC_RELAXED, __HIP_MEMORY_SCOPE_AGENT);
  };

  auto do_round = [&](const unsigned R, const unsigned round) -> bool {
    __syncthreads();
    for (int s = tid; s <= HSK; s += TBP) {
      hkey[s] = EMPTY_KEY; hrow[s] = 0; hocc[s] = 0;
      if constexpr (!DD) hval[s] = 0;
      if constexpr (!UQ && !DD) hhint[s] = 0;
    }
    if (tid == 0) { lnu = 0; lsent = 0; lnext = 0; }
    __syncthreads();
    unsigned csrc[EB];
    unsigned short cslot[EB];
    bool cin[EB];
    const bool cached = (R == 1 && E <= (unsigned)(EB * TBP));
    for (unsigned x0 = 0; x0 < E; x0 += EB * TBP) {
      unsigned ge[EB];
      long long key[EB];
      unsigned ea[EB], rw[EB], hi[EB], sr[EB];
#pragma unroll
      for (int k = 0; k < EB; ++k) {
        const unsigned x = x0 + k * TBP + tid;
        ge[k] = x < E ? (unsigned)seg_entry(tpre, tstart, NT, x) : 0xFFFFFFFFu;
      }
#pragma unroll
      for (int k = 0; k < EB; ++k) {
        key[k] = 0; ea[k] = 0; rw[k] = 0; hi[k] = 0; sr[k] = 0;
        if (ge[k] != 0xFFFFFFFFu) {
          key[k] = w.ent_key[ge[k]]; ea[k] = w.ent_a[ge[k]]; rw[k] = w.ent_b[ge[k]]; hi[k] = w.ent_base[ge[k]];
          if (cached) sr[k] = w.ent_rec[ge[k]];
        }
      }
#pragma unroll
      for (int k = 0; k < EB; ++k) {
        if (x0 == 0) { csrc[k] = sr[k]; cslot[k] = 0; cin[k] = false; }
        if (ge[k] == 0xFFFFFFFFu || !in_round(key[k], R, round)) continue;
        if (lnu >= (unsigned)UCAPK) continue;
        bool first;
        const unsigned h = lds_key_slot<HSK>(hkey, &lsent, key[k], true, &first);
        if (first) {
          const unsigned u = atomicAdd(&lnu, 1u);
          if (u < (unsigned)UCAPK) ulist[u] = (unsigned short)h;
        }
        if constexpr (UQ) atomicAdd(&hval[h], a.sparse_unique ? (ea[k] & 0xFFFFu) : (ea[k] >> 16));
        else if constexpr (!DD) { if (mode == PA_LOOKUP) atomicAdd(&hval[h], ea[k] >> 16); }
        atomicAdd(&hocc[h], 1u);
        atomicMax(&hrow[h], rw[k]);
        if constexpr (!UQ && !DD) { if (hi[k]) atomicMax(&hhint[h], hi[k]); }
        if (x0 == 0) { cslot[k] = (unsigned short)h; cin[k] = true; }
      }
    }
    __syncthreads();
    if (lnu >= (unsigned)UCAPK) return true;
    KV_STAMPP(1);
    const unsigned nu = lnu;
    const unsigned lkeys_before = lkeys;
    __syncthreads();
    if (tid == 0) {
      lkeys += nu;
      if ((UQ && !a.sparse_unique) || DN) lbase = atomicAdd(&w.ctr[0], nu);
    }

    constexpr int PERU = (UCAPK + TBP - 1) / TBP;
    unsigned nhot, ncold;
    {
      unsigned kcnt[PERU];
      unsigned sum = 0, ch = 0, hh = 0;
#pragma unroll
      for (int q = 0; q < PERU; ++q) {
        const unsigned u = tid * PERU + q;
        kcnt[q] = u < nu ? hocc[ulist[u]] : 0u;
        sum += kcnt[q];
        if (u < nu) {
          if (kcnt[q] == 1u) ch += 1u;
          else if (kcnt[q] == 2u) ch += 1u << 10;
          else if (kcnt[q] <= (unsigned)LCOLD) ch += 1u << 20;
          else hh += 1u;
        }
      }
      unsigned tot, chtot, htot;
      unsigned run = block_excl_scan<NW>(sum, wtot, &tot);
      unsigned chrun = block_excl_scan<NW>(ch, wtot, &chtot);
      unsigned hrn = block_excl_scan<NW>(hh, wtot, &htot);
      const unsigned t1 = chtot & 1023u, t2 = (chtot >> 10) & 1023u;
      nhot = htot; ncold = nu - htot;
#pragma unroll
      for (int q = 0; q < PERU; ++q) {
        const unsigned u = tid * PERU + q;
        if (u < nu) {
          const unsigned s = ulist[u];
          unsigned rank;
          if (kcnt[q] == 1u) { rank = nhot + (chrun & 1023u); chrun += 1u; }
          else if (kcnt[q] == 2u) { rank = nhot + t1 + ((chrun >> 10) & 1023u); chrun += 1u << 10; }
          else if (kcnt[q] <= (unsigned)LCOLD) { rank = nhot + t1 + t2 + (chrun >> 20); chrun += 1u << 20; }
          else { rank = hrn; hrn += 1u; }
          kord[rank] = (unsigned short)s;
          hocc[s] = run; run += kcnt[q];
          hcn[s] = (unsigned short)kcnt[q];
          if (UQ) {
            const unsigned num = a.sparse_unique ? pbase + lkeys_before + u : lbase + u;
            hrow[s] = num;
            a.out_keys[num] = (s == (unsigned)HSK) ? EMPTY_KEY : hkey[s];
            if (a.sparse_unique) a.out_counts[num] = (int)hval[s];
            else if (a.out_counts) a.out_counts[num] = (int)(hval[s] > 65535u ? 65535u : hval[s]);
          }
          if (DN) {
            const unsigned num = lbase + u;
            hrow[s] = num;
            a.out_keys[num] = (s == (unsigned)HSK) ? EMPTY_KEY : hkey[s];
          }
        }
      }
    }
    __syncthreads();
    if (UQ && a.route_world > 0) {
      if (tid < MAXW) rh[tid] = 0;
      __syncthreads();
      unsigned rd[PERU], rr[PERU];
#pragma unroll
      for (int q = 0; q < PERU; ++q) {
        const unsigned u = tid * PERU + q;
        rd[q] = 0xFFFFFFFFu; rr[q] = 0;
        if (u < nu) {
          const unsigned s = ulist[u];
          const long long key = (s == (unsigned)HSK) ? EMPTY_KEY : hkey[s];
          rd[q] = owner_rank(key, a.route_world, a.route_rule);
          rr[q] = atomicAdd(&rh[rd[q]], 1u);
        }
      }
      __syncthreads();
      if (tid < a.route_world) rbase[tid] = rh[tid] ? atomicAdd(&a.route_gcount[tid], rh[tid]) : 0u;
      __syncthreads();
#pragma unroll
      for (int q = 0; q < PERU; ++q) {
        const unsigned u = tid * PERU + q;
        if (u < nu) {
          const unsigned s = ulist[u];
          const unsigned num = hrow[s];
          const unsigned at = rbase[rd[q]] + rr[q];
          if (at < a.route_C) {
            const size_t slot = (size_t)rd[q] * (a.route_C + 1) + 1 + at;
            a.route_seg[2 * slot] = (s == (unsigned)HSK) ? EMPTY_KEY : hkey[s];
            a.route_seg[2 * slot + 1] = (long long)(int)hval[s];
            a.route_slot_of[num] = (int)slot;
          } else {
            a.route_slot_of[num] = 0;
            atomicExch(a.route_overflow, 1u);
          }
        }
      }
    }

    {
      constexpr bool numbers = UQ || DN;
      auto file = [&](unsigned pos, unsigned src) { if (in_lds) lsrc[pos] = src; else gsrc[pos] = src; };
      if (a.det) {
        const int wave = tid >> 6, wl = tid & 63;
        for (unsigned x0 = 0; x0 < E; x0 += TBP) {
          const unsigned x = x0 + tid;
          bool valid = x < E;
          size_t ge = 0;
          unsigned h = 0xFFFFFFFFu;
          if (valid) {
            ge = seg_entry(tpre, tstart, NT, x);
            const long long key = w.ent_key[ge];
            valid = in_round(key, R, round);
            if (valid) { bool first; h = lds_key_slot<HSK>(hkey, &lsent, key, false, &first); }
          }
          unsigned within = 0;
          for (int j = 0; j < 63; ++j) {
            const unsigned hj = __shfl(h, j);
            if (j < wl && hj == h) within += 1u;
          }
          unsigned pos = 0;
          for (int wv = 0; wv < NW; ++wv) {
            if (wave == wv && valid) { pos = hocc[h] + within; atomicAdd(&hocc[h], 1u); }
            __syncthreads();
          }
          if (valid) { file(pos, w.ent_rec[ge]); if (numbers) w.ent_b[ge] = hrow[h]; }
        }
      } else if (cached) {
#pragma unroll
        for (int k = 0; k < EB; ++k)
          if (cin[k]) {
            file(atomicAdd(&hocc[cslot[k]], 1u), csrc[k]);
            if (numbers) w.ent_b[seg_entry(tpre, tstart, NT, (unsigned)(k * TBP + tid))] = hrow[cslot[k]];
          }
      } else {
        for (unsigned x = tid; x < E; x += TBP) {
          const size_t ge = seg_entry(tpre, tstart, NT, x);
          const long long key = w.ent_key[ge];
          const unsigned src = w.ent_rec[ge];
          if (!in_round(key, R, round)) continue;
          bool first;
          const unsigned h = lds_key_slot<HSK>(hkey, &lsent, key, false, &first);
          file(atomicAdd(&hocc[h], 1u), src);
          if (numbers) w.ent_b[ge] = hrow[h];
        }
      }
    }
    if (!in_lds) __threadfence_block();
    __syncthreads();
    KV_STAMPP(2);

    unsigned tid2 = threadIdx.x;
    asm volatile("" : "+v"(tid2));
    const int wl = (int)(tid2 & 63u), lane = wl % LPR, g = wl / LPR;
    const float* const gbase = a.grad;
    const float* const ebase = a.epart;
    const float* const gself = w.grad_self;
    int eoff[K];
    bool evalid[K];
  #pragma unroll
    for (int k = 0; k < K; ++k) { const int e0 = (lane + k * LPR) * V; evalid[k] = e0 < D; eoff[k] = evalid[k] ? e0 : 0; }
    const bool fast = !two_slots(OPT) && a.tv.single != 0u && a.ts0.single != 0u && a.use_hints != 0 &&
                      (a.tv.track_delta | a.ts0.track_delta) == 0u && a.use_mirror != 0;
    float* const vrows = a.tv.c0.rows;
    RowMeta* const vmeta = a.tv.c0.meta;
    float* const srows = a.ts0.c0.rows;
    const int SD = a.ts0.dim;
    const unsigned smax = a.ts0.max_rows, thr = a.tv.enter_threshold;
    const bool need_vmeta = keeps_var_flags(OPT) || thr != 0u;
    const unsigned mepoch = a.mirror_epoch & 0xFFFFu;
    constexpr int NS0 = slot0_blocks(OPT);

    const unsigned nbatch = (ncold + (unsigned)G - 1u) / (unsigned)G;
    const unsigned nitems = nhot + nbatch;
    KV_STAMPPV(6, E); KV_STAMPPV(7, nu); KV_STAMPPV(8, nhot);
#ifdef KV_PA_X_NOAPPLY
    return false;
#endif
    if (UQ) return false;
#ifdef KV_STAMPS
    unsigned long long st_t0 = wall_clock64(), st_hot = 0, st_cold = 0, st_nh = 0, st_nc = 0;
#endif
    for (;;) {
#ifdef KV_STAMPS
      const unsigned long long st_a = wall_clock64();
#endif
      unsigned it = 0;
      if (wl == 0) it = atomicAdd(&lnext, 1u);
      it = (unsigned)__builtin_amdgcn_readfirstlane((int)it);
      if (it >= nitems) break;
      int eo[K];
#pragma unroll
      for (int k = 0; k < K; ++k) { eo[k] = eoff[k]; asm volatile("" : "+v"(eo[k])); }
      int lane_i = lane;
      asm volatile("" : "+v"(lane_i));
      auto load_row = [&](unsigned pos, float (&dst)[K][V]) {
        const float* base = (pos & EP_TAG) ? ebase : (pos - w.self_lo < w.self_len) ? gself : gbase;
        const float* src = base + (size_t)(pos & ~EP_TAG) * D;
#pragma unroll
        for (int k = 0; k < K; ++k) ldv_stream<V>(src + eo[k], dst[k]);
      };
#ifdef KV_PA_X_NOHOT
      const bool is_hot = false;
#else
      const bool is_hot = it < nhot;
#endif
      const unsigned kr = is_hot ? it : nhot + (it - nhot) * (unsigned)G + (unsigned)g;
      const bool have = is_hot || kr < nu;
      const unsigned s = kord[have ? kr : nhot + (it - nhot) * (unsigned)G];
      const long long key = (s == (unsigned)HSK) ? EMPTY_KEY : hkey[s];
      const unsigned cnt = have ? (unsigned)hcn[s] : 0u;
      const unsigned st = hocc[s] - (unsigned)hcn[s];
      const unsigned rww = hrow[s];
      unsigned row = rww & ROW_MASK;
      const bool isnew = have && mode != PA_NONE && (rww & NEW_BIT) != 0u;
      unsigned hint = 0u, fsum = 0u;
      if constexpr (!UQ && !DD) { hint = isnew ? 0u : hhint[s]; fsum = hval[s]; }
      const bool live = is_hot ? g == 0 : have;
      if (__builtin_expect(__ballot(isnew) != 0ull, 0)) {
        unsigned r2 = row;
        if (isnew && lane == 0 && live) {
          Entry* e = table_entry_of(a.tv, key);
          if (e) {
            if (r2 == 0u) { const unsigned er = load_entry(e).row; r2 = er != ROW_TOMB ? er : 0u; }
            e->hint = 0u;
          }
        }
        if (LPR > 1) r2 = __shfl(r2, 0, LPR);
// ... 28 lines not shown
          }
          hint_loaded = false; have_x = true; have_s = hh != 0u;
        } else {
          if (st_live && !isnew) vm = load_freq_flags(a.tv, row);
          uint4 rq = make_uint4((unsigned)key, (unsigned)((unsigned long long)key >> 32), st_live ? row : 0u, st_live ? hint : 0u);
          prefetch_state<OPT, V, LPR, K>(a, rq, st_live, lane_i, D, m0, hint_loaded, pre, have_x, have_s);
          if (!have_x) {
#pragma unroll
            for (int k = 0; k < K; ++k)
#pragma unroll
              for (int cc = 0; cc < V; ++cc) pre.x[k][cc] = 0.f;
          }
        }
      };
      constexpr bool dedup = DD;
      if (is_hot) {
        const unsigned lo = st, hi = st + cnt;
        constexpr int SR = G * RB;
        const unsigned nst = (cnt + SR - 1) / SR;
        auto ldpos = [&](unsigned stp, unsigned (&pp)[RB]) {
#pragma unroll
          for (int j = 0; j < RB; ++j) {
            const unsigned idx = lo + stp * SR + j * G + g;
            pp[j] = src_at(idx < hi ? idx : lo);
          }
        };
        unsigned pa_[RB], pb_[RB];
        float va[RB][K][V];
        ldpos(0, pa_);
        if (!dedup) prefetch();
        for (unsigned stp = 0; stp < nst; ++stp) {
#pragma unroll
          for (int j = 0; j < RB; ++j) load_row(pa_[j], va[j]);
          ldpos(stp + 1, pb_);
#pragma unroll
          for (int j = 0; j < RB; ++j) {
            const bool ok = lo + stp * SR + j * G + g < hi;
#pragma unroll
            for (int k = 0; k < K; ++k)
#pragma unroll
              for (int cc = 0; cc < V; ++cc) gv[k][cc] += ok ? va[j][k][cc] : 0.f;
            pa_[j] = pb_[j];
          }
        }
#pragma unroll
        for (int o = LPR; o < 64; o <<= 1) {
#pragma unroll
          for (int k = 0; k < K; ++k)
#pragma unroll
            for (int cc = 0; cc < V; ++cc) gv[k][cc] += __shfl_xor(gv[k][cc], o);
        }
      } else {
        float g2[K][V];
        const unsigned p0 = src_at(st < E ? st : 0u);
        const bool two = __ballot(live && cnt >= 2u) != 0ull;
        const unsigned p1 = src_at((cnt >= 2u ? st + 1u : st) < E ? (cnt >= 2u ? st + 1u : st) : 0u);
        load_row(p0, gv);
        if (two) load_row(p1, g2);
        if (!dedup) prefetch();
        if (two) {
#pragma unroll
          for (int k = 0; k < K; ++k)
#pragma unroll
            for (int cc = 0; cc < V; ++cc) gv[k][cc] += (cnt >= 2u) ? g2[k][cc] : 0.f;
        }
#ifndef KV_PA_RC
#define KV_PA_RC 4
#endif
        constexpr int RC = (KV_PA_RC / K) > 0 ? (KV_PA_RC / K) : 1;
        for (unsigned j0 = 2; __ballot(live && j0 < cnt) != 0ull; j0 += RC) {
          float val[RC][K][V];
          unsigned pj[RC];
#pragma unroll
          for (int j = 0; j < RC; ++j) pj[j] = src_at(j0 + j < cnt ? st + j0 + j : (st < E ? st : 0u));
#pragma unroll
          for (int j = 0; j < RC; ++j) load_row(pj[j], val[j]);
#pragma unroll
          for (int j = 0; j < RC; ++j) {
            const bool okj = j0 + j < cnt;
#pragma unroll
            for (int k = 0; k < K; ++k)
#pragma unroll
              for (int cc = 0; cc < V; ++cc) gv[k][cc] += okj ? val[j][k][cc] : 0.f;
          }
        }
      }

      if (dedup) {
        const bool direct = a.direct_rows > 0;
        if (live && (!direct || (unsigned long long)key < (unsigned long long)a.direct_rows)) {
          const size_t orow = direct ? (size_t)key : (size_t)(a.out_map ? a.out_map[row] : (int)row);
          float* dst = a.out_sum + orow * D;
#pragma unroll
          for (int k = 0; k < K; ++k)
            if (evalid[k]) stv<V>(dst + eo[k], gv[k]);
        }
        continue;
      }
      bool vnew = false;
      if (mode != PA_NONE) {
        const bool nk = st_live && isnew;
        if (__builtin_expect(__ballot(nk) != 0ull, 0)) {
          if (nk) {
            const unsigned long long h = pick64((unsigned long long)key ^ (a.tv.seed * 0x9E3779B97F4A7C15ULL));
            const float* ia = a.tv.init_table + (size_t)((unsigned)h % a.tv.init_rows) * D;
            const float* ib = a.tv.init_table + (size_t)((unsigned)(h >> 32) % a.tv.init_rows) * D;
            float* xrow = row_ptr(a.tv, row);
#pragma unroll
            for (int k = 0; k < K; ++k) {
              float va_[V], vb_[V];
              ldv<V>(ia + eo[k], va_);
              ldv<V>(ib + eo[k], vb_);
#pragma unroll
              for (int cc = 0; cc < V; ++cc) pre.x[k][cc] = (va_[cc] + vb_[cc]) * 0.5f;
              if (evalid[k]) stv<V>(xrow + eo[k], pre.x[k]);
            }
            have_x = true;
          }
        }
        const unsigned oflags = nk ? (unsigned)FLAG_DIRTY : (vm.y & 0xFFu);
        const bool recompute = st_live && (mode == PA_LOOKUP ? (oflags & FLAG_DIRTY) != 0u : nk);
        bool big = false;
        if (__ballot(recompute) != 0ull) {
#pragma unroll
          for (int k = 0; k < K; ++k)
#pragma unroll
            for (int cc = 0; cc < V; ++cc) big |= recompute && evalid[k] && fabsf(pre.x[k][cc]) >= CUTOFF;
// ... 55 lines not shown
          unsigned lo16 = (sfreq & 0xFFFFu) + 1u;
          if (lo16 > 65535u) lo16 = 65535u;
          mp->freq = (a.day << 16) | lo16;
          mp->state = (unsigned char)MIRROR_DIRTY;
        }
        opt_core<OPT, V, LPR, K>(vrows + (size_t)rr * D, srows + (size_t)h2 * SD, nullptr, &vmeta[(size_t)rr * META_STRIDE].flags,
                                 &mp->flags, nullptr, act, false, D, gv, a.opt, lane_i, pre.x, pre.s);
        general = fin_live && !ok;
      }
#ifndef KV_PA_X_NOGENERAL
      if (!fast || __ballot(general) != 0ull)
        finish_key<MODE_APPLY, OPT, V, LPR, K>(a, ra, general, hint_loaded && general, m0, gv, lane_i, &pre, have_x && general,
                                               have_s && general);
#endif
#ifdef KV_STAMPS
      {
        const unsigned long long now = wall_clock64();
        if (is_hot) { st_hot += now - st_a; ++st_nh; } else { st_cold += now - st_a; ++st_nc; }
      }
#endif
    }
#ifdef KV_STAMPS
    if (wl == 0) {
      unsigned long long* d = w.dbg + (size_t)(8192 + blockIdx.x * NW + (tid >> 6)) * 16;
      d[0] = st_t0; d[1] = wall_clock64(); d[2] = st_hot; d[3] = st_cold; d[4] = st_nh; d[5] = st_nc;
    }
#endif
    __syncthreads();
    KV_STAMPP(3);
    return false;
  };
  if (do_round(1u, 0u)) {
    __syncthreads();
    if (tid == 0) { stkR[0] = 2; stkr[0] = 0; stkR[1] = 2; stkr[1] = 1; sp = 2; }
    __syncthreads();
    while (sp > 0) {
      const unsigned R = stkR[sp - 1], round = stkr[sp - 1];
      __syncthreads();
      if (tid == 0) --sp;
      const bool ovf = do_round(R, round);
      __syncthreads();
      if (ovf && tid == 0) {
        if (sp + 2 <= 24) {
          stkR[sp] = 2 * R; stkr[sp] = round; ++sp;
          stkR[sp] = 2 * R; stkr[sp] = round + R; ++sp;
        } else {
          raise_error(a.tv, 2u);
        }
      }
      __syncthreads();
    }
  }
  if (tid == 0 && mode != PA_NONE && !DD) atomicAdd(&w.ctr[5], lkeys);
}

__device__ __forceinline__ void papply_route_tail(const PartArgs& a, const int mode_, const unsigned nblocks) {
  if ((mode_ & 0xFF) != PA_UNIQUE || a.route_world <= 0 || a.route_need == nullptr) return;
  __shared__ unsigned rt_last, rt_tot, rt_max;
  __syncthreads();
  if (threadIdx.x == 0) {
    rt_last = __hip_atomic_fetch_add(&a.route_gcount[MAXW], 1u, __ATOMIC_RELAXED, __HIP_MEMORY_SCOPE_AGENT) == nblocks - 1u ? 1u : 0u;
    rt_tot = 0u; rt_max = 0u;
  }
  __syncthreads();
  if (!rt_last) return;
  const int d = (int)threadIdx.x;
  if (d < a.route_world) {
    const unsigned c = __hip_atomic_load(&a.route_gcount[d], __ATOMIC_RELAXED, __HIP_MEMORY_SCOPE_AGENT);
    __hip_atomic_store(&a.route_gcount[d], 0u, __ATOMIC_RELAXED, __HIP_MEMORY_SCOPE_AGENT);
    a.route_seg[2 * (size_t)d * (a.route_C + 1)] = c < a.route_C ? c : a.route_C;
    a.route_seg[2 * (size_t)d * (a.route_C + 1) + 1] = 0;
    atomicMax(&rt_max, c);
    atomicAdd(&rt_tot, c);
  }
  __syncthreads();
  if (d == 0) {
    __hip_atomic_store(&a.route_gcount[MAXW], 0u, __ATOMIC_RELAXED, __HIP_MEMORY_SCOPE_AGENT);
    *a.route_need = rt_max;
    if (a.route_uhint) __hip_atomic_store(a.route_uhint, rt_tot, __ATOMIC_RELAXED, __HIP_MEMORY_SCOPE_SYSTEM);
  }
}

template <int OPT, int V, int LPR, int K, int TBP>
__global__ void __launch_bounds__(TBP, KV_PA_WAVES) k_papply(WsDev w, PartArgs a, int mode) {
  papply_body<OPT, V, LPR, K, TBP>(w, a, mode);
}

template <int TBP>
__global__ void __launch_bounds__(TBP, KV_PA_WAVES) k_papply_uniq(WsDev w, PartArgs a, int mode) {
  papply_body<OPT_ADAM_V4, 4, 1, 1, TBP, PA_UNIQUE>(w, a, mode);
  papply_route_tail(a, mode, gridDim.x);
}
#ifndef KV_PD_WAVES
#define KV_PD_WAVES 6
#endif
template <int V, int LPR, int K, int TBP, bool NUM = false>
__global__ void __launch_bounds__(TBP, TBP >= 512 ? KV_PD_WAVES : KV_PA_WAVES) k_papply_dedup(WsDev w, PartArgs a) {
  papply_body<OPT_ADAGRAD, V, LPR, K, TBP, NUM ? PA_DEDUP_NUM : PA_DEDUP>(w, a, PA_DEDUP);
}
template <int V, int LPR, int K>
__global__ void __launch_bounds__(256, KV_PA_WAVES) k_papply_dedup_multi(const MultiDesc* __restrict__ descs) {
  const MultiDesc& m = descs[blockIdx.y];
  if (blockIdx.x >= m.w.P || m.n == 0) return;
  papply_body<OPT_ADAGRAD, V, LPR, K, 256, PA_DEDUP>(m.w, m.a, PA_DEDUP);
}
__global__ void __launch_bounds__(256, KV_PA_WAVES) k_papply_uniq_multi(const MultiDesc* __restrict__ descs, int mode) {
  const MultiDesc& m = descs[blockIdx.y];
  if (blockIdx.x >= m.w.P || m.n == 0) return;
  papply_body<OPT_ADAM_V4, 4, 1, 1, 256, PA_UNIQUE>(m.w, m.a, mode);
  papply_route_tail(m.a, mode, m.w.P);
}
template <int OPT, int V, int LPR, int K>
__global__ void __launch_bounds__(256, KV_PA_WAVES) k_papply_multi(const MultiDesc* __restrict__ descs, int mode) {
  const MultiDesc& m = descs[blockIdx.y];
  if (blockIdx.x >= m.w.P || m.n == 0) return;
  papply_body<OPT, V, LPR, K, 256>(m.w, m.a, mode);
}

template <int OPT>
int launch_papply_t(const WsDev& wd, const PartArgs& pa, int mode, hipStream_t s, const MultiDesc* md = nullptr, int ntab = 0) {
  const int D = pa.tv.dim;
  const size_t sh = (size_t)wd.ntiles * 4 + 32;
  if ((D & 3) != 0 || (mode & 0xFF) > PA_NONE) return KV_UNIMPLEMENTED;
#define KV_PA(V, LPR, K)                                                     \
  do {                                                                       \
    if (md) k_papply_multi<OPT, V, LPR, K><<<dim3(wd.P, (unsigned)ntab), 256, sh, s>>>(md, mode);   \
    else if (wd.P <= 512u && !pa.det) k_papply<OPT, V, LPR, K, 512><<<(int)wd.P, 512, sh, s>>>(wd, pa, mode);   \
    else k_papply<OPT, V, LPR, K, 256><<<(int)wd.P, 256, sh, s>>>(wd, pa, mode);       \
    return KV_OK;                                                            \
  } while (0)
  const int q = D / 4;
  if (q <= 1) KV_PA(4, 1, 1);
  if (q <= 2) KV_PA(4, 2, 1);
  if (q <= 4) KV_PA(4, 4, 1);
  if (q <= 8) KV_PA(4, 8, 1);
  if (q <= 16) KV_PA(4, 8, 2);
  if (q <= 32) KV_PA(4, 16, 2);
  if (q <= 64) KV_PA(4, 64, 1);
#undef KV_PA
  return KV_UNIMPLEMENTED;
}
```

tfplus_amd/csrc/kv_types.h:

```cpp
#pragma once

#include <hip/hip_runtime.h>

namespace __attribute__((visibility("hidden"))) kvhip_internal {

enum Mode { MODE_LOOKUP = 0, MODE_APPLY = 1, MODE_DEDUP = 2, MODE_SCATTER = 3, MODE_MARK = 4, MODE_UNIQUE = 5,
            MODE_APPLYIDX = 6 };
enum Opt { OPT_ADAM_V4 = 0, OPT_ADAM_V3 = 1, OPT_ADAGRAD = 2, OPT_FTRL = 3, OPT_FTRL_V2 = 4, OPT_GROUP_FTRL_V2 = 5 };
constexpr bool group_adam(int opt) { return opt == OPT_ADAM_V4 || opt == OPT_ADAM_V3; }
constexpr bool two_slots(int opt) { return opt == OPT_FTRL || opt == OPT_FTRL_V2 || opt == OPT_GROUP_FTRL_V2; }
constexpr bool keeps_var_flags(int opt) { return opt == OPT_ADAGRAD || opt == OPT_FTRL_V2; }
constexpr int slot0_blocks(int opt) { return group_adam(opt) ? 3 : 1; }

struct __attribute__((aligned(16))) Entry {
  long long key;
  unsigned row;
  unsigned hint;
};

struct RowMeta {
  long long key;
  unsigned freq;
  unsigned char flags;
  unsigned char delta;
// ... 16 lines not shown

struct Chunk {
  float* rows;
  RowMeta* meta;
};

struct TableDev {
  Chunk c0;
  Entry* entries;
  unsigned long long mask;
  Chunk* chunks;
  int chunk_bits;
  unsigned* counters;
  const unsigned* free_rows;
  unsigned max_rows;
  const float* init_table;
  unsigned init_rows;
  int dim;
  unsigned enter_threshold;
  unsigned long long seed;
  unsigned track_delta;
  unsigned* err_host;
  unsigned single;
};

struct WsDev {
  long long* ent_key;
  unsigned* ent_a;
  unsigned* ent_b;
  unsigned* ent_base;
  unsigned* ent_rec;
  unsigned* toff;
  unsigned* slot_rank;
  unsigned* order;
  uint4* coldlist;
  uint4* hotlist;
  uint4* litem;
  uint4* pmeta;
  uint4* items;
  float* hpart;
  unsigned* ctr;
  unsigned ntiles, P;
  int pshift;
  unsigned seg_cap;
  int* zero_counts;
  unsigned long long* dbg;
  unsigned* mrow;
  unsigned* mcount;
  float* epart;
  unsigned self_lo, self_len;
  const void* ids_self;
  const float* grad_self;
  unsigned short* pos_ent;
};

struct OptArgs {
  float lr, b1p, b2p, b1, b2, eps, l1, l2, l21, l2s, lr_power;
  float alpha, l21_norm;
  int update_slots;
  int fast;
};

struct PartArgs {
  TableDev tv, ts0, ts1;
  OptArgs opt;
  const float* grad;
  unsigned day;
  int scatter_op, is_insert;
  int mark_what;
  const unsigned* fvals;
  long long* out_keys;
  float* out_sum;
  const int* out_map;
  int* out_counts;
  int count_once;
  long long direct_rows;
  int use_hints;
  int fold_op;
  int det;
  int sparse_unique;
  long long n;
  const float* epart;
  unsigned day_lk;
  int route_world, route_rule;
  unsigned route_C;
  long long* route_seg;
  int* route_slot_of;
  unsigned* route_overflow;
  unsigned* route_gcount;
  unsigned* route_need;
  unsigned* route_uhint;
  unsigned uniq_serial;
  int use_mirror;
  unsigned mirror_epoch;
  int dd_number;
};

struct MultiDesc {
  WsDev w;
  PartArgs a;
  const void* ids;
  const int* counts;
  float* out;
  long long n;
};
enum PaMode { PA_LOOKUP = 0, PA_APPLYIDX = 1, PA_NONE = 2, PA_UNIQUE = 3, PA_DEDUP = 4,
              PA_DEDUP_NUM = 5 };
// ... 3 lines not shown
```

tfplus_amd/csrc/kvhip.hip:

```cpp

#include <hip/hip_runtime.h>

#include <algorithm>
#include <atomic>
#include <cmath>
#include <cstdarg>
#include <cstdint>
#include <cstdio>
#include <cstring>
#include <ctime>
#include <mutex>
#include <string>
#include <vector>
#include <unordered_set>

#include "kv_host.h"

using namespace kvhip_internal;

namespace {

#include "kv_device.h"
#include "kv_kernels.h"
#include "kv_fused.h"
// ... 201 lines not shown
    }
  }
  t->rows_ub += (unsigned long long)extra;
  t->idx_ub += (unsigned long long)extra;
  return KV_OK;
}

unsigned pick_partitions(long long n, bool many_distinct = false) {
  if (many_distinct && n >= (1ll << 18)) {
    const unsigned P0 = pick_partitions(n, false);
    return P0 < (unsigned)MAX_P ? P0 * 2u : P0;
  }
  unsigned long long want = std::min<unsigned long long>(1024, (unsigned long long)((n + 31) / 32));
  want = std::max<unsigned long long>(want, (unsigned long long)((n + 1023) / 1024));
  unsigned P = 1;
  while (P < want && P < (unsigned)MAX_P) P <<= 1;
  return P;
}

unsigned fused_default_P(long long n) {
  unsigned P = 64;
  while ((long long)P * 384 < n && P < 1024u) P <<= 1;
  return std::min(P, pick_partitions(n, false));
}

size_t chunk_cap(long long n) { return (size_t)(n / HC + n / (LCOLD + 1) + 4); }

bool stream_is_capturing(hipStream_t s) {
  hipStreamCaptureStatus cap = hipStreamCaptureStatusNone;
  return hipStreamIsCapturing(s, &cap) == hipSuccess && cap != hipStreamCaptureStatusNone;
}
int ws_sync(hipStream_t s) {
  if (stream_is_capturing(s))
    return fail(KV_FAILED_PRECONDITION, "the table's batch workspace has to grow for this call, which needs a stream synchronisation: "
                                        "run the op once with this batch length outside the stream capture first");
  HIP_TRY(hipStreamSynchronize(s));
  return KV_OK;
}
int ensure_workspace(kv_table* t, long long n, bool need_part, hipStream_t s) {
  Workspace& w = t->ws;
  const unsigned P = pick_partitions(n, true);
  int rc;
  if (n > w.cap_n || P > w.capP) {
    if ((rc = ws_sync(s))) return rc;
    long long cap = std::max<long long>(n, TILE);
    if (w.cap_n) cap = std::max<long long>(cap, std::min<long long>(w.cap_n * 2, 1ll << 30));
    cap = (cap + TILE - 1) / TILE * TILE;
    const unsigned capP = std::max(pick_partitions(cap, true), P);
    const size_t nt = (size_t)(cap / TILE);
    w.cap_n = 0; w.capP = 0; w.hpart_elems = 0; w.epart_elems = 0;
    t->batch_serial = 0;
    if ((rc = regrow(&w.ent_key, (size_t)cap)) || (rc = regrow(&w.ent_a, (size_t)cap)) ||
        (rc = regrow(&w.ent_b, (size_t)cap)) || (rc = regrow(&w.ent_base, (size_t)cap)) || (rc = regrow(&w.ent_rec, (size_t)cap)) ||
        (rc = regrow(&w.toff, nt * (capP + 1))) || (rc = regrow(&w.slot_rank, (size_t)cap)) ||
        (rc = regrow(&w.order, (size_t)cap + 1)) || (rc = regrow(&w.coldlist, 2 * (size_t)cap)) ||
        (rc = regrow(&w.hotlist, 2 * (size_t)cap)) || (rc = regrow(&w.litem, (size_t)cap)) ||
        (rc = regrow(&w.items, (size_t)cap)) || (rc = regrow(&w.pmeta, (size_t)capP + 1)) ||
        (rc = regrow(&w.mcount, nt + 1)))
      return rc;
    if (!w.ctr) {
      HIP_TRY(hipMalloc(&w.ctr, 8 * sizeof(unsigned)));
      HIP_TRY(hipMemset(w.ctr, 0, 8 * sizeof(unsigned)));
    }
#ifdef KV_STAMPS
    if ((rc = regrow(&w.dbg, (size_t)16384 * 16))) return rc;
    hipMemset(w.dbg, 0, (size_t)16384 * 16 * 8);
#endif
    w.cap_n = cap;
    w.capP = capP;
  }
  const long long pe = (long long)chunk_cap(w.cap_n) * (long long)t->dim;
  if (need_part && w.hpart_elems < pe) {
    if ((rc = ws_sync(s))) return rc;
    w.hpart_elems = 0;
    if ((rc = regrow(&w.hpart, (size_t)pe))) return rc;
    w.hpart_elems = pe;
  }
  const long long ee = ((n + TILE - 1) / TILE) * (long long)(TILE / 2) * (long long)t->dim;
  if (need_part && w.epart_elems < ee) {
    if ((rc = ws_sync(s))) return rc;
    const long long want = std::max(ee, std::min((w.cap_n / 2) * (long long)t->dim, w.epart_elems + w.epart_elems / 2));
    w.epart_elems = 0;
    if ((rc = regrow(&w.epart, (size_t)want))) return rc;
    w.epart_elems = want;
  }
  return KV_OK;
}

int ensure_pos_ent(kv_table* t, long long n, hipStream_t s) {
  Workspace& w = t->ws;
  if (w.pos_cap >= n) return KV_OK;
  int rc;
  if ((rc = ws_sync(s))) return rc;
  const long long cap = std::max<long long>(n, w.cap_n);
  w.pos_cap = 0;
  if ((rc = regrow(&w.pos_ent, (size_t)cap))) return rc;
  w.pos_cap = cap;
  return KV_OK;
}

WsDev ws_view(kv_table* t, long long n, const SelfSegment* self) {
  Workspace& w = t->ws;
  WsDev d;
  d.ent_key = w.ent_key; d.ent_a = w.ent_a; d.ent_b = w.ent_b; d.ent_base = w.ent_base; d.ent_rec = w.ent_rec;
  d.toff = w.toff;
  d.slot_rank = w.slot_rank;
  d.order = w.order;
  d.coldlist = w.coldlist;
  d.hotlist = w.hotlist;
  d.litem = w.litem;
  d.items = w.items;
  d.pmeta = w.pmeta;
  d.hpart = w.hpart;
  d.ctr = w.ctr;
  d.ntiles = (unsigned)((n + TILE - 1) / TILE);
  use_partitions(d, pick_partitions(n));
  d.seg_cap = 0;
  d.zero_counts = nullptr;
  d.dbg = w.dbg;
  d.mrow = w.slot_rank;
  d.mcount = w.mcount;
  d.epart = w.epart;
  d.pos_ent = nullptr;
  d.self_lo = d.self_len = 0; d.ids_self = nullptr; d.grad_self = nullptr;
  if (self) { d.self_lo = self->lo; d.self_len = self->len; d.ids_self = self->ids; d.grad_self = self->grad; }
  return d;
}


bool fast_math_on(const kv_table* t) { return t->fast_math && !t->deterministic; }
int det_mode(const kv_table* t) { return t->occurrence_order ? 2 : t->deterministic ? 1 : 0; }

unsigned today(const kv_table* t) {
  if (t->fixed_day >= 0) return (unsigned)t->fixed_day & 0xFFFFu;
  return (unsigned)(std::time(nullptr) / (3600 * 24)) & 0xFFFFu;
}

template <bool FIRST>
void launch_tile(kv_table* t, const WsDev& wd, const void* ids, const int* counts, long long n, hipStream_t s,
                 int ids_kind, const MultiDesc* md, int ntab, unsigned gx) {
  if (ids_kind < 0) ids_kind = t->key_dtype == KV_DT_INT32 ? 1 : 0;
  const int grid = (int)wd.ntiles;
  const size_t sh = tile_smem_bytes(FIRST);
  const int det = det_mode(t);
#define KV_TILE(IDT)                                                                     \
  do {                                                                                   \
    if (md) k_tile_multi<FIRST, IDT><<<dim3(gx, (unsigned)ntab), TBT, sh, s>>>(md);       \
    else k_tile<FIRST, IDT><<<grid, TBT, sh, s>>>(wd, (const IDT*)ids, counts, n, det);  \
  } while (0)
  if (ids_kind == 2) {
    if constexpr (!FIRST) KV_TILE(IdCount);
  } else if (ids_kind == 1) KV_TILE(int);
  else KV_TILE(long long);
#undef KV_TILE
}

void launch_gather(const TableDev& td, const WsDev& wd, float* op, long long m, hipStream_t s,
                   const MultiDesc* md, int ntab, bool order) {
  const int D = td.dim;
  const int q = (D % 4 == 0) ? D / 4 : 0;
  const bool vec = q > 0 && (q & (q - 1)) == 0 && q <= TB;
  const long long rows_per_block = vec ? TB / q : 1;
  constexpr int gcap = 8192;
  const int grid = vec ? nblocks(m, q <= 64 ? TB : (int)rows_per_block, gcap) : nblocks(m * D, TB, 4096);
#define KV_GATHER(VQ)                                                                        \
  do {                                                                                       \
    if (md) k_gather_multi<VQ><<<dim3((unsigned)grid, (unsigned)ntab), TB, 0, s>>>(md);       \
    else if (order) k_gather<VQ, true><<<grid + ITEM_BLOCKS, TB, 0, s>>>(td, wd, op, m);      \
    else k_gather<VQ, false><<<grid, TB, 0, s>>>(td, wd, op, m);                              \
  } while (0)
  switch (vec ? q : 0) {
    case 1: KV_GATHER(1); break;
    case 2: KV_GATHER(2); break;
    case 4: KV_GATHER(4); break;
    case 8: KV_GATHER(8); break;
    case 16: KV_GATHER(16); break;
    case 32: KV_GATHER(32); break;
    case 64: KV_GATHER(64); break;
    case 128: KV_GATHER(128); break;
// ... 200 lines not shown
  return mirror_on_entry(t, s, keep);
}

int join_side(kv_table* t, hipStream_t s) {
  int rc;
  if (t->part_pending) {
    if ((rc = hop_behind_last(t, s)) || (rc = flush_part(t, s))) return rc;
  }
  if ((t->mirror_var || t->mirror_slot) && (rc = hop_behind_last(t, s))) return rc;
  return mirror_on_entry(t, s, KEEP_NONE);
}

int enter_op(kv_table* t, hipStream_t s, unsigned keep, bool settle, bool mutates) {
  int rc;
  if ((rc = report_deferred_error(t, s))) return rc;
  return hand_over(t, s, keep, settle, mutates);
}

template <int MODE>
void index_pass(kv_table* t, const WsDev& wd, const PartArgs& pa, const void* ids, const int* counts, long long n,
                int ids_kind, float* out, hipStream_t s, bool file_order) {
  t->fused_index = false;
  {
    ProfScope ps(t, MODE == MODE_LOOKUP ? KV_PROF_LOOKUP_TILE : KV_PROF_INDEX, s);
    launch_tile<false>(t, wd, ids, counts, n, s, ids_kind);
  }
  {
    ProfScope ps(t, MODE == MODE_LOOKUP ? KV_PROF_LOOKUP_PART : KV_PROF_INDEX, s);
    launch_part_keys<MODE>(wd, pa, s);
  }
  ProfScope ps(t, MODE == MODE_LOOKUP ? KV_PROF_LOOKUP_ORDER : KV_PROF_INDEX, s);
  if (MODE == MODE_LOOKUP && out) launch_gather(pa.tv, wd, out, n, s, nullptr, 0, file_order);
  else launch_order(pa.tv, wd, n, s);
}

void choose_partitions(kv_table* t, WsDev& wd, long long n) {
  {
    const unsigned u_prev = t->err_host ? reinterpret_cast<volatile unsigned*>(t->err_host)[1] : 0u;
    const bool hinted = !t->deterministic && t->batch_n_prev == n && u_prev > 0u;
    t->batch_n_prev = n;
    if (hinted) {
      const unsigned long long u = std::min<unsigned long long>(u_prev, (unsigned long long)n);
      const unsigned long long per = 256ull;
      const unsigned long long want = std::max<unsigned long long>((u + per - 1ull) / per, (unsigned long long)((n + 2047) / 2048));
      const unsigned pmax = std::min<unsigned>((unsigned)MAX_P, std::max(64u, t->ws.capP));
      unsigned P = 64;
      while (P < want && P < pmax) P <<= 1;
      wd.P = P;
    } else {
      wd.P = fused_default_P(n);
    }
    wd.pshift = 64 - ilog2(wd.P);
    t->index_P = wd.P;
  }
}

int fused_lookup_pass(kv_table* t, WsDev& wd, const PartArgs& pa, const void* ids, const int* counts, long long n,
                      int ids_kind, float* out, hipStream_t s, bool defer_part) {
  t->fused_index = true;
  choose_partitions(t, wd, n);
  {
    ProfScope ps(t, KV_PROF_LOOKUP_TILE, s);
    launch_ltile(t, pa.tv, wd, ids, counts, n, out, s, ids_kind);
  }
  if (defer_part) {
    set_pending_part(t, wd, pa);
    return KV_OK;
  }
  ProfScope ps(t, KV_PROF_LOOKUP_PART, s);
  launch_part2(wd, pa, s);
  return KV_OK;
}

std::mutex g_tables_mu;
std::unordered_set<kv_table*> g_tables;
void retire_stream(hipStream_t dead) {
  std::lock_guard<std::mutex> l(g_tables_mu);
  for (kv_table* t : g_tables) {
    std::lock_guard<std::mutex> lt(t->mu);
    if (t->has_last && t->last_stream == dead) { t->has_last = false; t->last_stream = nullptr; }
  }
}

std::atomic<uint64_t> g_serial{0};
std::atomic<uint64_t> g_uid{0};

BatchStage g_stage[64][2];

int stage_take(BatchStage& st, size_t bytes, StageSlot** out) {
  st.mu.lock();
  StageSlot& sl = st.slot[st.cursor++ & 3u];
  if (sl.consumed && hipEventSynchronize(sl.consumed) != hipSuccess) {
    st.mu.unlock();
    return fail(KV_INTERNAL, "descriptor staging: event sync failed");
  }
  if (sl.cap < bytes) {
    if (sl.host) hipHostFree(sl.host);
    if (sl.dev) hipFree(sl.dev);
    sl.host = sl.dev = nullptr;
    sl.cap = std::max<size_t>(bytes, 64 * 1024);
    if (hipHostMalloc(&sl.host, sl.cap) != hipSuccess || hipMalloc(&sl.dev, sl.cap) != hipSuccess ||
        (!sl.consumed && hipEventCreateWithFlags(&sl.consumed, hipEventDisableTiming) != hipSuccess)) {
      sl.cap = 0;
      st.mu.unlock();
      return fail(KV_RESOURCE_EXHAUSTED, "descriptor staging: allocation failed");
    }
  }
  *out = &sl;
  return KV_OK;
}

int check_same_shape(int num_tables, const kv_handle_t* tables, const char* what) {
  int rc;
// ... 82 lines not shown
  t->key_dtype = key_dtype;
  t->dim = dim;
  t->enter_threshold = (unsigned)(unsigned short)std::min<int>(enter_threshold, 65535);
  unsigned long long hint = capacity_hint > 0 ? (unsigned long long)capacity_hint + 1 : 0;
  t->chunk_bits = std::max(16, std::min(30, ilog2(std::max<unsigned long long>(hint, 1))));
  hipStream_t s = nullptr;
  int rc = KV_OK;
  do {
    if (hipMalloc(&t->d_chunks, MAX_CHUNKS * sizeof(Chunk)) != hipSuccess ||
        hipMalloc(&t->d_counters, 8 * sizeof(unsigned)) != hipSuccess ||
        hipMalloc(&t->d_stat, 4 * sizeof(unsigned long long)) != hipSuccess) {
      rc = fail(KV_RESOURCE_EXHAUSTED, "hipMalloc of table header failed");
      break;
    }
    if (hipHostMalloc(&t->err_host, 4 * sizeof(unsigned), hipHostMallocMapped) != hipSuccess ||
        hipEventCreateWithFlags(&t->last_done, hipEventDisableTiming) != hipSuccess) {
      rc = fail(KV_RESOURCE_EXHAUSTED, "table header: pinned word / event");
      break;
    }
    t->err_host[0] = t->err_host[1] = t->err_host[2] = t->err_host[3] = 0;
    t->uid = ++g_uid;
    unsigned init[8] = {1, 0, 0, 0, 0, 0, 0, 0};
    if (hipMemcpy(t->d_counters, init, sizeof init, hipMemcpyHostToDevice) != hipSuccess) {
      rc = fail(KV_INTERNAL, "hipMemcpy failed");
      break;
    }
    if ((rc = add_chunk(t, s))) break;
    if ((rc = build_index(t, pow2ceil(std::max<unsigned long long>(2 * t->rows_cap, 1024)), 1, s))) break;
  } while (0);
  if (rc) { kv_destroy(t); return rc; }
  { std::lock_guard<std::mutex> l(g_tables_mu); g_tables.insert(t); }
  *out = t;
  return KV_OK;
}

int kv_destroy(kv_handle_t t) {
  if (!t) return KV_OK;
  { std::lock_guard<std::mutex> l(g_tables_mu); g_tables.erase(t); }
  {
    DeviceGuard dgm(t->device);
    if (t->mirror_slot) mirror_unpair(t, nullptr, t);
    if (t->mirror_var) { t->mirror_var->mirror_dirty.store(false); t->mirror_var->mirror_slot = nullptr; t->mirror_var = nullptr; }
  }
  DeviceGuard dg(t->device);
  hipDeviceSynchronize();
  for (auto& c : t->chunks) { hipFree(c.rows); hipFree(c.meta); }
  hipFree(t->entries); hipFree(t->d_chunks); hipFree(t->d_counters); hipFree(t->d_stat); hipFree(t->free_rows);
  hipFree(t->init_table);
  hipFree(t->route_hist);
  for (auto e : t->ev) hipEventDestroy(e);
  Workspace& w = t->ws;
  hipFree(w.ent_key); hipFree(w.ent_a); hipFree(w.ent_b); hipFree(w.ent_base); hipFree(w.ent_rec); hipFree(w.toff); hipFree(w.slot_rank);
  hipFree(w.order); hipFree(w.coldlist); hipFree(w.hotlist); hipFree(w.litem); hipFree(w.items); hipFree(w.pmeta); hipFree(w.hpart);
  hipFree(w.mcount); hipFree(w.epart); hipFree(w.pos_ent);
  hipFree(w.ctr); hipFree(w.dbg); hipFree(w.scat_keys); hipFree(w.scat_sum); hipFree(w.seg_off);
  if (t->err_host) hipHostFree(t->err_host);
  if (t->cnt_host) hipHostFree(t->cnt_host);
  if (t->last_done) hipEventDestroy(t->last_done);
  delete t;
  return KV_OK;
}

int kv_reserve(kv_handle_t t, int64_t capacity) {
  int rc;
  if ((rc = check_table(t))) return rc;
  DeviceGuard dg(t->device);
  std::lock_guard<std::mutex> l(t->mu);
  if ((rc = settle_pending(t))) return rc;
  unsigned long long save = t->rows_ub, save_idx = t->idx_ub;
  long long extra = capacity + 1 - (long long)t->rows_ub;
  if (extra <= 0) return KV_OK;
  rc = ensure_capacity(t, extra, nullptr);
  t->rows_ub = std::min(save, t->rows_ub);
  t->idx_ub = std::min(save_idx, t->idx_ub);
  return rc;
}

int kv_init_table(kv_handle_t t, const float* table, int64_t rows, kv_stream_t stream) {
  int rc;
  if ((rc = check_table(t))) return rc;
  if (!table || rows <= 0) return fail(KV_INVALID_ARGUMENT, "random_initializer must be a non-empty [rows, dim] matrix");
  DeviceGuard dg(t->device);
  std::lock_guard<std::mutex> l(t->mu);
  if (t->initialized && t->init_table && !t->init_placeholder) return KV_OK;
  if ((rc = settle_pending(t))) return rc;
  if (t->init_table) { HIP_TRY(hipStreamSynchronize((hipStream_t)stream)); hipFree(t->init_table); t->init_table = nullptr; }
  HIP_TRY(hipMalloc(&t->init_table, (size_t)rows * t->dim * sizeof(float)));
  HIP_TRY(hipMemcpyAsync(t->init_table, table, (size_t)rows * t->dim * sizeof(float),
                         hipMemcpyDeviceToDevice, (hipStream_t)stream));
  t->init_rows = rows;
  t->init_placeholder = false;
  t->initialized = true;
  return KV_OK;
}

int kv_is_initialized(kv_handle_t t, int* out) {
  int rc;
  if ((rc = check_table(t))) return rc;
  *out = t->initialized ? 1 : 0;
  return KV_OK;
}

int kv_set_clock_days(kv_handle_t t, int day) {
  int rc;
  if ((rc = check_table(t))) return rc;
  t->fixed_day = day;
  ++t->op_serial;
  return KV_OK;
}
int kv_set_seed(kv_handle_t t, uint64_t seed) {
  int rc;
  if ((rc = check_table(t))) return rc;
  DeviceGuard dg(t->device);
  std::lock_guard<std::mutex> l(t->mu);
  if ((rc = settle_pending(t))) return rc;
  t->seed = seed;
  return KV_OK;
}

int kv_set_deterministic(kv_handle_t t, int on) {
  int rc;
  if ((rc = check_table(t))) return rc;
  DeviceGuard dg(t->device);
  std::lock_guard<std::mutex> l(t->mu);
  if ((rc = settle_pending(t))) return rc;
  if (on < 0 || on > 2) return fail(KV_INVALID_ARGUMENT, "kv_set_deterministic: on = %d (0, 1 or 2)", on);
  if (on == 2 && t->shard_refs.load() > 0)
    return fail(KV_UNIMPLEMENTED, "kv_set_deterministic(h, 2): the table serves a kv_shard (occurrence order is a single-table notion)");
  t->deterministic = on != 0;
  t->occurrence_order = on == 2;
  t->batch_serial = 0;
  t->fused_index = false;
  return KV_OK;
}

int kv_set_fast_math(kv_handle_t t, int on) {
  int rc;
  if ((rc = check_table(t))) return rc;
  std::lock_guard<std::mutex> l(t->mu);
  t->fast_math = on != 0;
  return KV_OK;
}

int kv_get_stat(kv_handle_t t, int which, int64_t* value) {
  int rc;
  if ((rc = check_table(t))) return rc;
  if (!value) return fail(KV_INVALID_ARGUMENT, "kv_get_stat: null value");
  std::lock_guard<std::mutex> l(t->mu);
  if (which == KV_STAT_MIRROR_APPLIES) { *value = t->stat_mirror_applies; return KV_OK; }
  if (which == KV_STAT_MIRROR_EPOCHS) { *value = t->stat_mirror_epochs.load(); return KV_OK; }
  return fail(KV_INVALID_ARGUMENT, "kv_get_stat: unknown counter %d", which);
}

int kv_prepare_capture(kv_handle_t t, int64_t max_new_ids, kv_stream_t stream) {
  int rc;
  if ((rc = check_table(t))) return rc;
  if (max_new_ids < 0) return fail(KV_INVALID_ARGUMENT, "max_new_ids < 0");
  TableOp op(t, stream);
  hipStream_t s = op.s;
  if ((rc = enter_op(t, s))) return rc;
  mirror_ban(t, s);
  unsigned c[3];
  HIP_TRY(hipMemcpyAsync(c, t->d_counters, sizeof c, hipMemcpyDeviceToHost, s));
  HIP_TRY(hipStreamSynchronize(s));
  if (c[1]) return flagged_error(t, c[1], s);
  const long long freed = std::max(0, (int)c[2]);
  t->rows_ub = c[0];
  t->free_known = freed;
  t->idx_ub = t->idx_base + (c[0] - t->bump_base) +
              (unsigned long long)std::max<long long>(0, (long long)t->pushes_since - (freed - t->free_base));
  const unsigned long long r0 = t->rows_ub, i0 = t->idx_ub;
  if ((rc = ensure_capacity(t, max_new_ids, s))) return rc;
  t->rows_ub = r0; t->idx_ub = i0;
  HIP_TRY(hipStreamSynchronize(s));
  return KV_OK;
}

int kv_profile_enable(kv_handle_t t, int max_launches) {
  int rc;
  if ((rc = check_table(t))) return rc;
  DeviceGuard dg(t->device);
  std::lock_guard<std::mutex> l(t->mu);
  for (auto e : t->ev) hipEventDestroy(e);
  t->ev.clear();
  t->ev_kind.clear();
  t->ev_used = 0;
  t->prof = max_launches > 0;
  for (int i = 0; i < 2 * max_launches; ++i) {
    hipEvent_t e;
    HIP_TRY(hipEventCreate(&e));
    t->ev.push_back(e);
  }
  t->ev_kind.assign((size_t)std::max(max_launches, 0), 0);
  return KV_OK;
}

int kv_profile_select(kv_handle_t t, unsigned kind_mask) {
  int rc;
  if ((rc = check_table(t))) return rc;
  std::lock_guard<std::mutex> l(t->mu);
  t->prof_mask = kind_mask;
  return KV_OK;
}

int kv_profile_sample(kv_handle_t t, int every) {
  int rc;
  if ((rc = check_table(t))) return rc;
  if (every < 1) return fail(KV_INVALID_ARGUMENT, "kv_profile_sample: every %d", every);
  std::lock_guard<std::mutex> l(t->mu);
  t->prof_every = every;
  for (unsigned& q : t->prof_seq) q = 0;
  return KV_OK;
}

// ... 28 lines not shown
```

tfplus_amd/kv_variable/python/ops/gen_kv_variable_ops.py:

```python
import ctypes

import numpy as np
import torch

from tfplus_amd import _lib

_TORCH_KEY = {torch.int64: _lib.KV_DT_INT64, torch.int32: _lib.KV_DT_INT32}


class KvHandle(object):

  def __init__(self, ptr, dim, key_dtype, value_dtype, device, enter_threshold, name):
    self.ptr = ptr
    self.dim = dim
    self.key_dtype = key_dtype
    self.value_dtype = value_dtype
    self.device = device
    self.enter_threshold = enter_threshold
    self.name = name
    self.batch = None

  def __del__(self):
    try:
      if self.ptr:
# ... 363 lines not shown
kv_variable_scatter_update_v2 = _scatter(0)
kv_variable_scatter_add_v2 = _scatter(1)
kv_variable_scatter_sub_v2 = _scatter(2)
kv_variable_scatter_mul_v2 = _scatter(3)
kv_variable_scatter_div_v2 = _scatter(4)
kv_variable_scatter_min_v2 = _scatter(5)
kv_variable_scatter_max_v2 = _scatter(6)


def kv_set_clock_days(table_handle, day):
  _lib.check(_lib.lib().kv_set_clock_days(table_handle.ptr, int(day)))


def kv_set_seed(table_handle, seed):
  _lib.check(_lib.lib().kv_set_seed(table_handle.ptr, int(seed)))


def kv_get_meta(table_handle, indices):
  ids = torch.as_tensor(indices, dtype=torch.int64).to(_dev(table_handle)).contiguous().view(-1)
  fw = torch.empty(ids.numel(), dtype=torch.int32, device=ids.device)
  fl = torch.empty(ids.numel(), dtype=torch.uint8, device=ids.device)
  _lib.check(_lib.lib().kv_get_meta(table_handle.ptr, _p(ids), ids.numel(), _p(fw), _p(fl),
                                    _stream(table_handle)))
  fw = fw.cpu().numpy().view(np.uint32)
  fl = fl.cpu().numpy()
  return [None if not (b & 0x80) else {"freq": int(w & 0xFFFF), "day": int(w >> 16),
                                       "blacklist": bool(b & 1), "under_threshold": bool(b & 2)}
          for w, b in zip(fw, fl)]


def kv_reserve(table_handle, capacity):
  _lib.check(_lib.lib().kv_reserve(table_handle.ptr, int(capacity)))


PROF_KINDS = ("lookup_tile", "lookup_part", "lookup_order", "apply_index", "apply_sorted", "apply_span", "apply_tsum",
              "apply_unique", "apply_tile")


def kv_attach_slot(var, slot):
  _lib.check(_lib.lib().kv_attach_slot(var.ptr, slot.ptr, _stream(var)))


KV_ORDER_ARRIVAL, KV_ORDER_FIXED, KV_ORDER_OCCURRENCE = 0, 1, 2


def kv_set_deterministic(table_handle, on=True):
  _lib.check(_lib.lib().kv_set_deterministic(table_handle.ptr, int(on)))


def kv_set_fast_math(table_handle, on=True):
  _lib.check(_lib.lib().kv_set_fast_math(table_handle.ptr, int(bool(on))))


KV_STAT_MIRROR_APPLIES, KV_STAT_MIRROR_EPOCHS = 0, 1


def kv_get_stat(table_handle, which):
  v = ctypes.c_int64(0)
  _lib.check(_lib.lib().kv_get_stat(table_handle.ptr, int(which), ctypes.byref(v)))
  return int(v.value)


def kv_forget_stream(stream):
  _lib.check(_lib.lib().kv_forget_stream(ctypes.c_void_p(stream.cuda_stream)))


def kv_prepare_capture(table_handle, max_new_ids):
  _lib.check(_lib.lib().kv_prepare_capture(table_handle.ptr, int(max_new_ids), _stream(table_handle)))


def kv_profile_enable(table_handle, max_launches):
  _lib.check(_lib.lib().kv_profile_enable(table_handle.ptr, int(max_launches)))


def kv_profile_select(table_handle, kinds=None):
  mask = 0xFFFFFFFF if kinds is None else sum(1 << PROF_KINDS.index(k) for k in kinds)
  _lib.check(_lib.lib().kv_profile_select(table_handle.ptr, mask))


def kv_profile_sample(table_handle, every=1):
  _lib.check(_lib.lib().kv_profile_sample(table_handle.ptr, int(every)))


def kv_profile_read(table_handle):
  n = len(PROF_KINDS)
  ms = (ctypes.c_double * n)()
  cnt = (ctypes.c_int64 * n)()
  _lib.check(_lib.lib().kv_profile_read(table_handle.ptr, ms, cnt, n))
  return {k: (ms[i], cnt[i]) for i, k in enumerate(PROF_KINDS)}


def kv_bucket_by_owner(table_handle, indices, world, n_dev=None, id_counts=None, with_payload=False, owner_rule=0):
  ids = _ids(table_handle, indices).reshape(-1)
  dev = _dev(table_handle)
  out = torch.empty(ids.numel(), dtype=torch.int64, device=dev)
  perm = torch.empty(ids.numel(), dtype=torch.int32, device=dev)
  counts = torch.empty(int(world), dtype=torch.int64, device=dev)
  pairs = pos = cin = None
  if with_payload:
    pairs = torch.empty((ids.numel(), 2), dtype=torch.int64, device=dev)
    pos = torch.empty(ids.numel(), dtype=torch.int32, device=dev)
    cin = None if id_counts is None else id_counts.to(torch.int32).contiguous()
  _lib.check(_lib.lib().kv_bucket_by_owner(table_handle.ptr, _p(ids), ids.numel(), _p(n_dev), int(world), int(owner_rule), _p(out),
                                           _p(perm), ctypes.c_void_p(counts.data_ptr()), _p(cin), _p(pairs), _p(pos),
                                           _stream(table_handle)))
  return (out, perm, counts, pairs, pos) if with_payload else (out, perm, counts)

# ... 501 lines not shown
```

Before: 7.872 billion ids/s (each id: 1 embedding lookup + 1 fused GroupAdam-V4 apply).

## Route heavy-hitter keys to a dedicated partition across fused lookup and apply

Adds a heavy-key routing scheme. Keys that the previous batch's apply identified as hot are published to a double-buffered device list. In the next lookup tile pass those keys go to an extra partition slot and their per-tile cell positions are recorded. The partition/apply kernels then reduce each heavy key's contributions across tiles with one owner block, so a Zipf-skewed hot key no longer makes a single partition's segment huge. This adds extra LDS probing, toff stride changes and bookkeeping, plus invalidation hooks on deterministic mode, capture, import and clear.

```diff
diff --git a/include/kvhip.h b/include/kvhip.h
--- a/include/kvhip.h
+++ b/include/kvhip.h
@@ -106,6 +106,7 @@
 
 #define KV_STAT_MIRROR_APPLIES 0
 #define KV_STAT_MIRROR_EPOCHS 1
+#define KV_STAT_HEAVY_ROUTED 2
 int kv_get_stat(kv_handle_t h, int which, int64_t* value);
 
 int kv_prepare_capture(kv_handle_t h, int64_t max_new_ids, kv_stream_t stream);
diff --git a/tfplus_amd/csrc/kv_apply.hip b/tfplus_amd/csrc/kv_apply.hip
--- a/tfplus_amd/csrc/kv_apply.hip
+++ b/tfplus_amd/csrc/kv_apply.hip
@@ -131,7 +131,8 @@
   bool pa_reuse = reuse;
   for (int i = 0; i < num_tables && reuse; ++i)
     if (ns[i] > 0) {
-      const bool held = tokens[i] != 0 && tokens[i] == vars[i]->batch_serial && ns[i] == vars[i]->batch_n && vars[i]->fused_index;
+      const bool held = tokens[i] != 0 && tokens[i] == vars[i]->batch_serial && ns[i] == vars[i]->batch_n && vars[i]->fused_index &&
+                        vars[i]->index_hv < 0;
       if (!held) reuse = false;
       if (!held || !vars[i]->part_pending) pa_reuse = false;
     }
@@ -181,7 +182,7 @@
   if (fz) {
     int pa_mode = pa_reuse ? PA_LOOKUP : PA_NONE;
     if (!reuse) {
-      for (int i = 0; i < num_tables; ++i) vars[i]->fused_index = true;
+      for (int i = 0; i < num_tables; ++i) { vars[i]->fused_index = true; vars[i]->index_hv = -1; }
       launch_ltile(vars[0], hd[0].a.tv, wmax, nullptr, nullptr, nmax, nullptr, s, -1, md, num_tables, false);
       pa_mode = PA_APPLYIDX;
       for (int i = 0; i < num_tables; ++i)
@@ -255,6 +256,7 @@
     if (pa_route) {
       v->fused_index = true;
       choose_partitions(v, wd, n);
+      if (!self) heavy_route(v, wd, s);
       tile_ids = ids;
       pa_mode = PA_APPLYIDX;
     } else {
@@ -266,6 +268,7 @@
     pa_mode = PA_NONE;
   }
   if (v->fused_index && reuse && v->index_P) use_partitions(wd, v->index_P);
+  if (v->fused_index) heavy_view(v, wd, true);
   if ((rc = mirror_decide(v, s0, pa, v->fused_index && !two_slots(OPT), s))) return rc;
   if (v->fused_index) rc = fused_apply<OPT>(v, wd, pa, n, s, pa_mode, tile_ids);
   else rc = launch_apply<MODE_APPLY, OPT>(v, wd, pa, n, s);
diff --git a/tfplus_amd/csrc/kv_device.h b/tfplus_amd/csrc/kv_device.h
--- a/tfplus_amd/csrc/kv_device.h
+++ b/tfplus_amd/csrc/kv_device.h
@@ -29,6 +29,10 @@
 constexpr int TILE = TBT * IPT;
 constexpr int LS = 2 * TILE;
 constexpr int MAX_P = 2048;
+constexpr int HEAVY_MAX = TBT < 512 ? TBT : 512;
+constexpr int HV_TILES = 512;
+constexpr unsigned HV_ABSENT = 0xFFFFu;
+constexpr int HV_PUB = 16;
 constexpr int MAX_CHUNKS = 32768;
 
 #ifdef KV_STAMPS
diff --git a/tfplus_amd/csrc/kv_fused.h b/tfplus_amd/csrc/kv_fused.h
--- a/tfplus_amd/csrc/kv_fused.h
+++ b/tfplus_amd/csrc/kv_fused.h
@@ -62,7 +62,7 @@
   b += (size_t)(LS + 1) * 4 + 16;
   b += (size_t)(LS + 1) * 2 + 16;
   b += (size_t)(TILE + 1) * 2 + 16;
-  b += (size_t)(MAX_P + 1) * 4 + 16;
+  b += (size_t)(MAX_P + 2) * 4 + 16;
   b += 64;
   return b;
 }
@@ -77,7 +77,7 @@
   s.lcnt = reinterpret_cast<unsigned*>(take((size_t)(LS + 1) * 4));
   s.lpos = reinterpret_cast<unsigned short*>(take((size_t)(LS + 1) * 2));
   s.lrun = reinterpret_cast<unsigned short*>(take((size_t)(TILE + 1) * 2));
-  s.hist = reinterpret_cast<unsigned*>(take((size_t)(MAX_P + 1) * 4));
+  s.hist = reinterpret_cast<unsigned*>(take((size_t)(MAX_P + 2) * 4));
   s.wtot = reinterpret_cast<unsigned*>(take(64));
   return s;
 }
@@ -103,6 +103,14 @@
   const unsigned P = w.P;
   constexpr bool PAIRS = std::is_same<IdT, IdCount>::value;
   const bool has_counts = PAIRS || counts != nullptr;
+  const unsigned HM = NOTABLE ? 0u : w.hv_max;
+  const unsigned PX = P + (HM ? 1u : 0u);
+  unsigned nh = 0;
+  long long hvk = EMPTY_KEY;
+  if (HM) {
+    nh = min(*w.hv_cnt, HM);
+    hvk = w.hv_keys[(unsigned)threadIdx.x < HM ? threadIdx.x : 0];
+  }
   KV_STAMP(0);
   KV_STAMP_HW(10);
 
@@ -165,12 +173,14 @@
     }
   };
   for (int s = tid; s <= LS; s += TBT) { sm.lkeys[s] = EMPTY_KEY; sm.lcnt[s] = 0; }
-  for (unsigned p = tid; p <= P; p += TBT) sm.hist[p] = 0;
+  for (unsigned p = tid; p <= PX; p += TBT) sm.hist[p] = 0;
+  for (unsigned i = tid; i < HM; i += TBT) sm.lrun[i] = (unsigned short)HV_ABSENT;
   if (tid == 0) lsent = 0;
   if (tile == 0 && tid == 0 && t.err_host)
     __hip_atomic_store(t.err_host + 1, w.ctr[5], __ATOMIC_RELAXED, __HIP_MEMORY_SCOPE_SYSTEM);
   lds_barrier();
   if (tile == 0 && tid < 8) w.ctr[tid] = 0;
+  if (HM && tile == 0 && tid == 0) *w.hv_next_cnt = 0u;
   if constexpr (PAIRS) {
 #pragma unroll
     for (int k = 0; k < IPT; ++k) {
@@ -306,31 +316,46 @@
   KV_STAMP(9);
   lds_barrier();
   KV_STAMP(1);
+  if (HM) {
+    if ((unsigned)tid < nh && hvk != EMPTY_KEY) {
+      unsigned h = (unsigned)(mix64((unsigned long long)hvk) >> 40) & (LS - 1);
+      for (;;) {
+        const long long kk = sm.lkeys[h];
+        if (kk == hvk) { sm.lcnt[h] += ((unsigned)tid + 1u) << 16; break; }
+        if (kk == EMPTY_KEY) break;
+        h = (h + 1) & (LS - 1);
+      }
+    }
+    lds_barrier();
+  }
 
   unsigned wcnt[IPT], wp[IPT], wr[IPT];
+  unsigned wh[IPT];
 #pragma unroll
   for (int k = 0; k < IPT; ++k) {
-    wcnt[k] = 0; wp[k] = 0; wr[k] = 0;
+    wcnt[k] = 0; wp[k] = 0; wr[k] = 0; wh[k] = 0;
     if ((win >> k) & 1u) {
-      wcnt[k] = sm.lcnt[tslot[k]];
-      wp[k] = part_of(kreg[k], w.pshift);
+      const unsigned lc = sm.lcnt[tslot[k]];
+      wcnt[k] = lc & 0xFFFFu;
+      wh[k] = lc >> 16;
+      wp[k] = wh[k] ? P : part_of(kreg[k], w.pshift);
       wr[k] = atomicAdd(&sm.hist[wp[k]], 1u | (wcnt[k] << 16)) & 0xFFFFu;
     }
   }
   lds_barrier();
   {
-    const unsigned per = (P + TBT - 1) / TBT;
-    const unsigned p0 = tid * per, p1 = min(p0 + per, P);
+    const unsigned per = (PX + TBT - 1) / TBT;
+    const unsigned p0 = tid * per, p1 = min(p0 + per, PX);
     unsigned sum = 0;
     for (unsigned p = p0; p < p1; ++p) sum += sm.hist[p];
     unsigned tot;
     unsigned run = block_excl_scan<TBT / 64, true>(sum, sm.wtot, &tot);
     for (unsigned p = p0; p < p1; ++p) { const unsigned c = sm.hist[p]; sm.hist[p] = run; run += c; }
-    if (tid == 0) sm.hist[P] = tot;
+    if (tid == 0) sm.hist[PX] = tot;
   }
   lds_barrier();
-  const unsigned nent = sm.hist[P] & 0xFFFFu;
-  for (unsigned p = tid; p <= P; p += TBT) w.toff[(size_t)tile * (P + 1) + p] = sm.hist[p];
+  const unsigned nent = sm.hist[PX] & 0xFFFFu;
+  for (unsigned p = tid; p <= PX; p += TBT) w.toff[(size_t)tile * (PX + 1) + p] = sm.hist[p];
   unsigned wpos[IPT];
 #pragma unroll
   for (int k = 0; k < IPT; ++k) {
@@ -338,6 +363,7 @@
     if ((win >> k) & 1u) {
       wpos[k] = (sm.hist[wp[k]] & 0xFFFFu) + wr[k];
       w.ent_key[(size_t)tile * TILE + wpos[k]] = kreg[k];
+      if (wh[k]) sm.lrun[wh[k] - 1u] = (unsigned short)wpos[k];
     }
   }
   if (det) {
@@ -369,6 +395,7 @@
   }
   lds_barrier();
   KV_STAMP(2);
+  for (unsigned i = tid; i < nh; i += TBT) w.hcell[(size_t)tile * HM + i] = sm.lrun[i];
 
   {
     constexpr unsigned PER = (TILE + 1 + TBT - 1) / TBT;
@@ -442,7 +469,7 @@
   }
 #pragma unroll
   for (int k = 0; k < IPT; ++k) {
-    if (tslot[k] == 0xFFFFFFFFu || sm.lcnt[tslot[k]] <= 1u) continue;
+    if (tslot[k] == 0xFFFFFFFFu || (sm.lcnt[tslot[k]] & 0xFFFFu) <= 1u) continue;
     const unsigned pre = sm.escan[sm.lpos[tslot[k]]];
     sm.mr[(pre & ES_POS) + myrank[k]] = (unsigned)(k * TBT + tid) | ((pre >> ES_NSH) << 11) | (myrank[k] == 0u ? 0x80000000u : 0u);
   }
@@ -491,7 +518,7 @@
     const unsigned t = tb + threadIdx.x;
     unsigned len = 0, s0 = 0;
     if (t < NT) {
-      const unsigned* c0 = w.toff + (size_t)t * (w.P + 1) + p;
+      const unsigned* c0 = w.toff + (size_t)t * toff_stride(w) + p;
       const unsigned a = c0[0], b = c0[1];
       s0 = a & 0xFFFFu;
       len = (b & 0xFFFFu) - s0;
@@ -509,13 +536,79 @@
   *pbase = pb;
   return run0;
 }
+template <int T>
+struct HeavyOwner {
+  static constexpr int HT = HV_TILES / T;
+  unsigned cell[HT];
+  unsigned ea[HT], eb[HT], eh[HT], es[HT];
+  long long key;
+  unsigned nh, first, n;
+
+  __device__ __forceinline__ void cells(const WsDev& w, unsigned p) {
+    key = EMPTY_KEY; nh = 0; first = 0; n = 0;
+#pragma unroll
+    for (int i = 0; i < HT; ++i) cell[i] = HV_ABSENT;
+    if (w.hv_max == 0u) return;
+    nh = min(*w.hv_cnt, w.hv_max);
+    if (p < nh) {
+      key = w.hv_keys[p];
+#pragma unroll
+      for (int i = 0; i < HT; ++i) {
+        const unsigned t = threadIdx.x * HT + i;
+        if (t < w.ntiles) cell[i] = w.hcell[(size_t)t * w.hv_max + p];
+      }
+    }
+  }
+  template <int NW>
+  __device__ __forceinline__ void settle(const WsDev& w, unsigned p, unsigned* wtot) {
+    if (w.hv_max == 0u || p >= nh) {
+#pragma unroll
+      for (int i = 0; i < HT; ++i) cell[i] = HV_ABSENT;
+      return;
+    }
+    unsigned c = 0;
+#pragma unroll
+    for (int i = 0; i < HT; ++i) {
+      if (cell[i] >= (unsigned)TILE) cell[i] = HV_ABSENT;
+      c += cell[i] != HV_ABSENT ? 1u : 0u;
+    }
+    first = block_excl_scan<NW>(c, wtot, &n);
+  }
+  __device__ __forceinline__ void entries(const WsDev& w, bool hints_sources) {
+#pragma unroll
+    for (int i = 0; i < HT; ++i) {
+      ea[i] = 0; eb[i] = 0; eh[i] = 0; es[i] = 0;
+      if (cell[i] != HV_ABSENT) {
+        const size_t ge = (size_t)(threadIdx.x * HT + i) * TILE + cell[i];
+        ea[i] = w.ent_a[ge]; eb[i] = w.ent_b[ge];
+        if (hints_sources) { eh[i] = w.ent_base[ge]; es[i] = w.ent_rec[ge]; }
+      }
+    }
+  }
+  __device__ __forceinline__ void reduce(unsigned* fsum, unsigned* row, unsigned* hint) const {
+    unsigned f = 0, r = 0, h = 0;
+#pragma unroll
+    for (int i = 0; i < HT; ++i) { f += ea[i] >> 16; r = max(r, eb[i]); h = max(h, eh[i]); }
+#pragma unroll
+    for (int o = 1; o < 64; o <<= 1) {
+      f += __shfl_xor(f, o); r = max(r, (unsigned)__shfl_xor(r, o)); h = max(h, (unsigned)__shfl_xor(h, o));
+    }
+    if ((threadIdx.x & 63) == 0) {
+      if (fsum && f) atomicAdd(fsum, f);
+      if (r) atomicMax(row, r);
+      if (hint && h) atomicMax(hint, h);
+    }
+  }
+};
+
 __device__ __forceinline__ void part2_body(const WsDev& w, const PartArgs& a) {
   constexpr int HSK = 1024;
   constexpr int UCAPK = HSK - TBK;
   constexpr int EB = 8;
-  __shared__ long long hkey[HSK + 1];
-  __shared__ unsigned hval[HSK + 1];
-  __shared__ unsigned hrow[HSK + 1];
+  constexpr unsigned HVS = HSK + 1;
+  __shared__ long long hkey[HSK + 2];
+  __shared__ unsigned hval[HSK + 2];
+  __shared__ unsigned hrow[HSK + 2];
   __shared__ unsigned short lnew[UCAPK + 8];
   __shared__ unsigned short ulist[UCAPK + 8];
   __shared__ unsigned lnu, lsent, lnnew, lkeys;
@@ -530,23 +623,33 @@
   const int D = a.tv.dim;
   KV_STAMPP(0);
   unsigned pbase;
+  HeavyOwner<TBK> hv;
+  hv.cells(w, p);
   const unsigned E = seg_directory_t<TBK, TBK / 64>(w, p, tpre, tstart, wtot, &pbase);
-  if (E == 0) return;
+  hv.settle<TBK / 64>(w, p, wtot);
+  if (E + hv.n == 0) return;
   __shared__ unsigned stkR[24], stkr[24];
   __shared__ int sp;
   if (tid == 0) { stkR[0] = 1; stkr[0] = 0; sp = 1; lkeys = 0; }
   __syncthreads();
-  if (E > 65535u) {
+  if (E + hv.n > 65535u) {
     if (tid == 0) raise_error(a.tv, 2u);
     return;
   }
+  hv.entries(w, false);
+  if (hv.n && tid == 0) atomicAdd(w.hv_stat, 1u);
   while (sp > 0) {
     const unsigned R = stkR[sp - 1], round = stkr[sp - 1];
     __syncthreads();
     if (tid == 0) --sp;
-    for (int s = tid; s <= HSK; s += TBK) { hkey[s] = EMPTY_KEY; hval[s] = 0; hrow[s] = 0; }
-    if (tid == 0) { lnu = 0; lsent = 0; lnnew = 0; }
+    const bool hvr = hv.n != 0u && in_round(hv.key, R, round);
+    for (int s = tid; s <= (int)HVS; s += TBK) { hkey[s] = EMPTY_KEY; hval[s] = 0; hrow[s] = 0; }
+    if (tid == 0) { lnu = hvr ? 1u : 0u; lsent = 0; lnnew = 0; if (hvr) ulist[0] = (unsigned short)HVS; }
     __syncthreads();
+    if (hvr) {
+      if (tid == 0) hkey[HVS] = hv.key;
+      hv.reduce(&hval[HVS], &hrow[HVS], nullptr);
+    }
     for (unsigned x0 = 0; x0 < E; x0 += EB * TBK) {
       unsigned ge[EB];
       long long key[EB];
diff --git a/tfplus_amd/csrc/kv_host.h b/tfplus_amd/csrc/kv_host.h
--- a/tfplus_amd/csrc/kv_host.h
+++ b/tfplus_amd/csrc/kv_host.h
@@ -57,6 +57,9 @@
   unsigned* seg_off = nullptr;
   long long seg_cap = 0;
   unsigned long long* dbg = nullptr;
+  long long* hv_keys = nullptr;
+  unsigned* hv_cnt = nullptr;
+  unsigned short* hcell = nullptr;
 };
 
 }
@@ -95,6 +98,9 @@
   bool fused_index = false;
   long long batch_n_prev = 0;
   unsigned index_P = 0;
+  int index_hv = -1;
+  int hv_cur = 0;
+  bool hv_banned = false;
   bool part_pending = false;
   unsigned char pend_wd[sizeof(WsDev)], pend_pa[sizeof(PartArgs)];
   long long stat_mirror_applies = 0;
@@ -325,11 +331,14 @@
 
 extern std::atomic<uint64_t> g_serial;
 void choose_partitions(kv_table* t, WsDev& wd, long long n);
+void heavy_route(kv_table* t, WsDev& wd, hipStream_t s);
+void heavy_view(kv_table* t, WsDev& wd, bool publish);
+int heavy_drop(kv_table* t, hipStream_t s);
 template <int MODE>
 void index_pass(kv_table* t, const WsDev& wd, const PartArgs& pa, const void* ids, const int* counts, long long n,
                 int ids_kind, float* out, hipStream_t s, bool file_order = true);
 int fused_lookup_pass(kv_table* t, WsDev& wd, const PartArgs& pa, const void* ids, const int* counts, long long n,
-                      int ids_kind, float* out, hipStream_t s, bool defer_part);
+                      int ids_kind, float* out, hipStream_t s, bool defer_part, bool heavy = false);
 template <int MODE, int OPT>
 int launch_apply(kv_table* prof_t, const WsDev& wd, const PartArgs& pa, long long nmax, hipStream_t s,
                  const MultiDesc* md = nullptr, int ntab = 0, bool skip_fin = false) {
diff --git a/tfplus_amd/csrc/kv_ops.hip b/tfplus_amd/csrc/kv_ops.hip
--- a/tfplus_amd/csrc/kv_ops.hip
+++ b/tfplus_amd/csrc/kv_ops.hip
@@ -173,6 +173,7 @@
   int rc;
   if ((rc = enter_op(t, s))) return rc;
   t->batch_serial = 0;
+  if ((rc = heavy_drop(t, s))) return rc;
   if ((rc = ensure_free_list(t, s))) return rc;
   HIP_TRY(hipMemsetAsync(t->d_stat, 0, 4 * sizeof(unsigned long long), s));
   with_id_type(t->key_dtype == KV_DT_INT32, [&](auto id) {
@@ -317,7 +318,8 @@
     PartArgs pa = self_part_args(t, m);
     pa.day = today(t);
     const bool defer_part = token != nullptr && n <= CHK;
-    if (fused_tab(t)) { if ((rc = fused_lookup_pass(t, wd, pa, idp, cp, m, pairs ? 2 : -1, op, s, defer_part))) return rc; }
+    const bool heavy = !pairs && !self && seg_cap == 0u;
+    if (fused_tab(t)) { if ((rc = fused_lookup_pass(t, wd, pa, idp, cp, m, pairs ? 2 : -1, op, s, defer_part, heavy))) return rc; }
     else index_pass<MODE_LOOKUP>(t, wd, pa, idp, cp, m, pairs ? 2 : -1, op, s, token != nullptr && n <= CHK);
   }
   HIP_TRY(hipGetLastError());
@@ -372,7 +374,7 @@
   if ((rc = hd.upload(s, &md))) return rc;
   kv_table* t0 = tables[0];
   if (fused_tab(t0)) {
-    for (int i = 0; i < num_tables; ++i) tables[i]->fused_index = true;
+    for (int i = 0; i < num_tables; ++i) { tables[i]->fused_index = true; tables[i]->index_hv = -1; }
     launch_ltile(t0, hd[0].a.tv, wmax, nullptr, nullptr, nmax, nullptr, s, ids_kind, md, num_tables, true);
     const bool defer = tokens != nullptr;
     if (!defer) launch_part2(wmax, hd[0].a, s, md, num_tables);
@@ -677,6 +679,7 @@
                                           "buffer sized from the count may be too small; count again");
     ++t->op_serial;
     t->batch_serial = 0;
+    if ((rc = heavy_drop(t, s))) return rc;
   }
   unsigned nrows = 1;
   if ((rc = stats(t, s, nullptr, &nrows))) return rc;
@@ -904,6 +907,7 @@
   t->gen += 1;
   t->slot_uid = 0;
   t->batch_serial = 0;
+  if ((rc = heavy_drop(t, s))) return rc;
   unsigned init[3] = {1, 0, 0};
   HIP_TRY(hipMemcpy(t->d_counters, init, sizeof init, hipMemcpyHostToDevice));
   launch_fill_entries(t, s);
diff --git a/tfplus_amd/csrc/kv_papply.h b/tfplus_amd/csrc/kv_papply.h
--- a/tfplus_amd/csrc/kv_papply.h
+++ b/tfplus_amd/csrc/kv_papply.h
@@ -19,12 +19,16 @@
   constexpr int G = 64 / LPR;
   constexpr int RB = (KV_PA_HOTRB / K) > 0 ? (KV_PA_HOTRB / K) : 1;
   constexpr int NW = TBP / 64;
-  __shared__ long long hkey[HSK + 1];
-  __shared__ unsigned hval[DD ? 1 : HSK + 1];
-  __shared__ unsigned hrow[HSK + 1];
-  __shared__ unsigned hhint[(UQ || DD) ? 1 : HSK + 1];
-  __shared__ unsigned hocc[HSK + 1];
-  __shared__ unsigned short hcn[HSK + 1];
+  constexpr bool HV = FM < 0;
+  constexpr unsigned HVS = HSK + 1;
+  __shared__ long long hkey[HSK + 2];
+  __shared__ unsigned hval[DD ? 1 : HSK + 2];
+  __shared__ unsigned hrow[HSK + 2];
+  __shared__ unsigned hhint[(UQ || DD) ? 1 : HSK + 2];
+  __shared__ unsigned hocc[HSK + 2];
+  __shared__ unsigned short hcn[HSK + 2];
+  __shared__ long long pubk[HV ? HV_PUB : 1];
+  __shared__ unsigned npub;
   __shared__ unsigned short ulist[UCAPK + 8];
   __shared__ unsigned short kord[UCAPK + 8];
   __shared__ unsigned lsrc[PA_LSRC];
@@ -36,6 +40,7 @@
   extern __shared__ __attribute__((aligned(16))) char smem_raw[];
   unsigned short* tpre = reinterpret_cast<unsigned short*>(smem_raw);
   unsigned short* tstart = tpre + w.ntiles;
+  unsigned* const hvl = reinterpret_cast<unsigned*>(tstart + w.ntiles);
 
   const int tid = threadIdx.x;
   const unsigned p = xcd_partition(blockIdx.x, w.P);
@@ -44,30 +49,51 @@
   const unsigned errflag = *reinterpret_cast<volatile unsigned*>(&a.tv.counters[1]);
   KV_STAMPP(0);
   unsigned pbase = 0;
+  HeavyOwner<TBP> hv;
+  if constexpr (HV) hv.cells(w, p);
   const unsigned E = seg_directory_t<TBP, NW>(w, p, tpre, tstart, wtot, &pbase);
+  unsigned EH = 0;
+  if constexpr (HV) { hv.template settle<NW>(w, p, wtot); EH = hv.n; }
+  const unsigned ET = E + EH;
   KV_STAMPP(5);
-  if (E == 0) return;
-  if (tid == 0) { sp = 0; lkeys = 0; }
+  if (ET == 0) return;
+  if (tid == 0) { sp = 0; lkeys = 0; npub = 0; }
   __syncthreads();
-  if (E > 65535u) {
+  if (ET > 65535u) {
     if (tid == 0) raise_error(a.tv, 2u);
     return;
   }
-  const bool in_lds = E <= (unsigned)PA_LSRC;
+  if constexpr (HV) {
+    hv.entries(w, true);
+    if (EH && tid == 0) atomicAdd(w.hv_stat, 1u);
+  }
+  const unsigned hv_min = max((unsigned)LCOLD + 1u, NT / 4u);
+  const bool in_lds = ET <= (unsigned)PA_LSRC;
+  unsigned ehr = 0;
   unsigned* const gsrc = w.order + pbase;
   auto src_at = [&](unsigned i) -> unsigned {
-    return in_lds ? lsrc[i] : __hip_atomic_load(gsrc + i, __ATOMIC_RELAXED, __HIP_MEMORY_SCOPE_AGENT);
+    if (in_lds) return lsrc[i];
+    if (HV && i < ehr) return hvl[i];
+    return __hip_atomic_load(gsrc + (i - ehr), __ATOMIC_RELAXED, __HIP_MEMORY_SCOPE_AGENT);
   };
 
   auto do_round = [&](const unsigned R, const unsigned round) -> bool {
     __syncthreads();
-    for (int s = tid; s <= HSK; s += TBP) {
+    const bool hvr = HV && EH != 0u && in_round(hv.key, R, round);
+    ehr = hvr ? EH : 0u;
+    for (int s = tid; s <= (int)HVS; s += TBP) {
       hkey[s] = EMPTY_KEY; hrow[s] = 0; hocc[s] = 0;
       if constexpr (!DD) hval[s] = 0;
       if constexpr (!UQ && !DD) hhint[s] = 0;
     }
-    if (tid == 0) { lnu = 0; lsent = 0; lnext = 0; }
-    __syncthreads();
+    if (tid == 0) { lnu = hvr ? 1u : 0u; lsent = 0; lnext = 0; if (hvr) ulist[0] = (unsigned short)HVS; }
+    __syncthreads();
+    if constexpr (HV) {
+      if (hvr) {
+        if (tid == 0) { hkey[HVS] = hv.key; hocc[HVS] = EH; }
+        hv.reduce(mode == PA_LOOKUP ? &hval[HVS] : nullptr, &hrow[HVS], &hhint[HVS]);
+      }
+    }
     unsigned csrc[EB];
     unsigned short cslot[EB];
     bool cin[EB];
@@ -155,6 +181,12 @@
           kord[rank] = (unsigned short)s;
           hocc[s] = run; run += kcnt[q];
           hcn[s] = (unsigned short)kcnt[q];
+          if constexpr (HV) {
+            if (w.hv_pub && kcnt[q] >= hv_min && s != (unsigned)HSK) {
+              const unsigned i = atomicAdd(&npub, 1u);
+              if (i < (unsigned)HV_PUB) pubk[i] = hkey[s];
+            }
+          }
           if (UQ) {
             const unsigned num = a.sparse_unique ? pbase + lkeys_before + u : lbase + u;
             hrow[s] = num;
@@ -211,7 +243,20 @@
 
     {
       constexpr bool numbers = UQ || DN;
-      auto file = [&](unsigned pos, unsigned src) { if (in_lds) lsrc[pos] = src; else gsrc[pos] = src; };
+      auto file = [&](unsigned pos, unsigned src) {
+        if (in_lds) lsrc[pos] = src;
+        else if (HV && pos < ehr) hvl[pos] = src;
+        else gsrc[pos - ehr] = src;
+      };
+      if constexpr (HV) {
+        if (hvr) {
+          unsigned at = hv.first;
+#pragma unroll
+          for (int i = 0; i < HeavyOwner<TBP>::HT; ++i)
+            if (hv.cell[i] != HV_ABSENT) file(at++, hv.es[i]);
+          if (tid == 0) hocc[HVS] = EH;
+        }
+      }
       if (a.det) {
         const int wave = tid >> 6, wl = tid & 63;
         for (unsigned x0 = 0; x0 < E; x0 += TBP) {
@@ -284,7 +329,7 @@
 
     const unsigned nbatch = (ncold + (unsigned)G - 1u) / (unsigned)G;
     const unsigned nitems = nhot + nbatch;
-    KV_STAMPPV(6, E); KV_STAMPPV(7, nu); KV_STAMPPV(8, nhot);
+    KV_STAMPPV(6, ET); KV_STAMPPV(7, nu); KV_STAMPPV(8, nhot);
 #ifdef KV_PA_X_NOAPPLY
     return false;
 #endif
@@ -419,9 +464,9 @@
         }
       } else {
         float g2[K][V];
-        const unsigned p0 = src_at(st < E ? st : 0u);
+        const unsigned p0 = src_at(st < ET ? st : 0u);
         const bool two = __ballot(live && cnt >= 2u) != 0ull;
-        const unsigned p1 = src_at((cnt >= 2u ? st + 1u : st) < E ? (cnt >= 2u ? st + 1u : st) : 0u);
+        const unsigned p1 = src_at((cnt >= 2u ? st + 1u : st) < ET ? (cnt >= 2u ? st + 1u : st) : 0u);
         load_row(p0, gv);
         if (two) load_row(p1, g2);
         if (!dedup) prefetch();
@@ -439,7 +484,7 @@
           float val[RC][K][V];
           unsigned pj[RC];
 #pragma unroll
-          for (int j = 0; j < RC; ++j) pj[j] = src_at(j0 + j < cnt ? st + j0 + j : (st < E ? st : 0u));
+          for (int j = 0; j < RC; ++j) pj[j] = src_at(j0 + j < cnt ? st + j0 + j : (st < ET ? st : 0u));
 #pragma unroll
           for (int j = 0; j < RC; ++j) load_row(pj[j], val[j]);
 #pragma unroll
@@ -601,6 +646,13 @@
     }
   }
   if (tid == 0 && mode != PA_NONE && !DD) atomicAdd(&w.ctr[5], lkeys);
+  if constexpr (HV) {
+    if (w.hv_pub && tid == 0 && npub != 0u) {
+      const unsigned np = min(npub, (unsigned)HV_PUB);
+      const unsigned base = atomicAdd(w.hv_next_cnt, np);
+      for (unsigned i = 0; i < np && base + i < w.hv_max; ++i) w.hv_next_keys[base + i] = pubk[i];
+    }
+  }
 }
 
 __device__ __forceinline__ void papply_route_tail(const PartArgs& a, const int mode_, const unsigned nblocks) {
@@ -669,7 +721,7 @@
 template <int OPT>
 int launch_papply_t(const WsDev& wd, const PartArgs& pa, int mode, hipStream_t s, const MultiDesc* md = nullptr, int ntab = 0) {
   const int D = pa.tv.dim;
-  const size_t sh = (size_t)wd.ntiles * 4 + 32;
+  const size_t sh = (size_t)wd.ntiles * 4 + 32 + (wd.hv_max ? (size_t)HV_TILES * 4 : 0);
   if ((D & 3) != 0 || (mode & 0xFF) > PA_NONE) return KV_UNIMPLEMENTED;
 #define KV_PA(V, LPR, K)                                                     \
   do {                                                                       \
diff --git a/tfplus_amd/csrc/kv_types.h b/tfplus_amd/csrc/kv_types.h
--- a/tfplus_amd/csrc/kv_types.h
+++ b/tfplus_amd/csrc/kv_types.h
@@ -92,7 +92,16 @@
   const void* ids_self;
   const float* grad_self;
   unsigned short* pos_ent;
+  unsigned hv_max;
+  int hv_pub;
+  const long long* hv_keys;
+  const unsigned* hv_cnt;
+  long long* hv_next_keys;
+  unsigned* hv_next_cnt;
+  unsigned short* hcell;
+  unsigned* hv_stat;
 };
+__host__ __device__ inline unsigned toff_stride(const WsDev& w) { return w.P + 1u + (w.hv_max ? 1u : 0u); }
 
 struct OptArgs {
   float lr, b1p, b2p, b1, b2, eps, l1, l2, l21, l2s, lr_power;
diff --git a/tfplus_amd/csrc/kvhip.hip b/tfplus_amd/csrc/kvhip.hip
--- a/tfplus_amd/csrc/kvhip.hip
+++ b/tfplus_amd/csrc/kvhip.hip
@@ -277,7 +277,7 @@
     t->batch_serial = 0;
     if ((rc = regrow(&w.ent_key, (size_t)cap)) || (rc = regrow(&w.ent_a, (size_t)cap)) ||
         (rc = regrow(&w.ent_b, (size_t)cap)) || (rc = regrow(&w.ent_base, (size_t)cap)) || (rc = regrow(&w.ent_rec, (size_t)cap)) ||
-        (rc = regrow(&w.toff, nt * (capP + 1))) || (rc = regrow(&w.slot_rank, (size_t)cap)) ||
+        (rc = regrow(&w.toff, nt * (capP + 2)))  || (rc = regrow(&w.slot_rank, (size_t)cap)) ||
         (rc = regrow(&w.order, (size_t)cap + 1)) || (rc = regrow(&w.coldlist, 2 * (size_t)cap)) ||
         (rc = regrow(&w.hotlist, 2 * (size_t)cap)) || (rc = regrow(&w.litem, (size_t)cap)) ||
         (rc = regrow(&w.items, (size_t)cap)) || (rc = regrow(&w.pmeta, (size_t)capP + 1)) ||
@@ -286,6 +286,11 @@
     if (!w.ctr) {
       HIP_TRY(hipMalloc(&w.ctr, 8 * sizeof(unsigned)));
       HIP_TRY(hipMemset(w.ctr, 0, 8 * sizeof(unsigned)));
+    }
+    if (!w.hv_cnt) {
+      HIP_TRY(hipMalloc(&w.hv_cnt, 4 * sizeof(unsigned)));
+      HIP_TRY(hipMemset(w.hv_cnt, 0, 4 * sizeof(unsigned)));
+      if ((rc = regrow(&w.hv_keys, (size_t)2 * HEAVY_MAX)) || (rc = regrow(&w.hcell, (size_t)HV_TILES * HEAVY_MAX))) return rc;
     }
 #ifdef KV_STAMPS
     if ((rc = regrow(&w.dbg, (size_t)16384 * 16))) return rc;
@@ -349,7 +354,36 @@
   d.pos_ent = nullptr;
   d.self_lo = d.self_len = 0; d.ids_self = nullptr; d.grad_self = nullptr;
   if (self) { d.self_lo = self->lo; d.self_len = self->len; d.ids_self = self->ids; d.grad_self = self->grad; }
+  d.hv_max = 0; d.hv_pub = 0;
+  d.hv_keys = nullptr; d.hv_cnt = nullptr; d.hv_next_keys = nullptr; d.hv_next_cnt = nullptr; d.hcell = nullptr; d.hv_stat = nullptr;
   return d;
+}
+
+void heavy_view(kv_table* t, WsDev& wd, bool publish) {
+  const Workspace& w = t->ws;
+  if (t->index_hv < 0 || !w.hv_cnt) return;
+  const int r = t->index_hv;
+  wd.hv_max = std::min<unsigned>(wd.P, (unsigned)HEAVY_MAX);
+  wd.hv_keys = w.hv_keys + (size_t)r * HEAVY_MAX;
+  wd.hv_cnt = w.hv_cnt + r;
+  wd.hv_next_keys = w.hv_keys + (size_t)(r ^ 1) * HEAVY_MAX;
+  wd.hv_next_cnt = w.hv_cnt + (r ^ 1);
+  wd.hcell = w.hcell;
+  wd.hv_stat = w.hv_cnt + 2;
+  wd.hv_pub = 0;
+  if (publish && t->index_hv == t->hv_cur) { wd.hv_pub = 1; t->hv_cur ^= 1; }
+}
+void heavy_route(kv_table* t, WsDev& wd, hipStream_t s) {
+  t->index_hv = -1;
+  if (t->deterministic || t->occurrence_order || t->hv_banned || !t->ws.hv_cnt) return;
+  if (wd.ntiles <= (unsigned)LCOLD || wd.ntiles > (unsigned)HV_TILES || stream_is_capturing(s)) return;
+  t->index_hv = t->hv_cur;
+  heavy_view(t, wd, false);
+}
+int heavy_drop(kv_table* t, hipStream_t s) {
+  t->batch_serial = 0;
+  if (t->ws.hv_cnt) HIP_TRY(hipMemsetAsync(t->ws.hv_cnt, 0, 2 * sizeof(unsigned), s));
+  return KV_OK;
 }
 
 
@@ -656,13 +690,15 @@
     }
     wd.pshift = 64 - ilog2(wd.P);
     t->index_P = wd.P;
+    t->index_hv = -1;
   }
 }
 
 int fused_lookup_pass(kv_table* t, WsDev& wd, const PartArgs& pa, const void* ids, const int* counts, long long n,
-                      int ids_kind, float* out, hipStream_t s, bool defer_part) {
+                      int ids_kind, float* out, hipStream_t s, bool defer_part, bool heavy) {
   t->fused_index = true;
   choose_partitions(t, wd, n);
+  if (heavy) heavy_route(t, wd, s);
   {
     ProfScope ps(t, KV_PROF_LOOKUP_TILE, s);
     launch_ltile(t, pa.tv, wd, ids, counts, n, out, s, ids_kind);
@@ -851,7 +887,7 @@
   Workspace& w = t->ws;
   hipFree(w.ent_key); hipFree(w.ent_a); hipFree(w.ent_b); hipFree(w.ent_base); hipFree(w.ent_rec); hipFree(w.toff); hipFree(w.slot_rank);
   hipFree(w.order); hipFree(w.coldlist); hipFree(w.hotlist); hipFree(w.litem); hipFree(w.items); hipFree(w.pmeta); hipFree(w.hpart);
-  hipFree(w.mcount); hipFree(w.epart); hipFree(w.pos_ent);
+  hipFree(w.mcount); hipFree(w.epart); hipFree(w.pos_ent); hipFree(w.hv_keys); hipFree(w.hv_cnt); hipFree(w.hcell);
   hipFree(w.ctr); hipFree(w.dbg); hipFree(w.scat_keys); hipFree(w.scat_sum); hipFree(w.seg_off);
   if (t->err_host) hipHostFree(t->err_host);
   if (t->cnt_host) hipHostFree(t->cnt_host);
@@ -930,6 +966,7 @@
   t->occurrence_order = on == 2;
   t->batch_serial = 0;
   t->fused_index = false;
+  if ((rc = heavy_drop(t, t->has_last ? t->last_stream : nullptr))) return rc;
   return KV_OK;
 }
 
@@ -948,6 +985,16 @@
   std::lock_guard<std::mutex> l(t->mu);
   if (which == KV_STAT_MIRROR_APPLIES) { *value = t->stat_mirror_applies; return KV_OK; }
   if (which == KV_STAT_MIRROR_EPOCHS) { *value = t->stat_mirror_epochs.load(); return KV_OK; }
+  if (which == KV_STAT_HEAVY_ROUTED) {
+    unsigned v = 0;
+    if (t->ws.hv_cnt) {
+      DeviceGuard dg(t->device);
+      HIP_TRY(hipDeviceSynchronize());
+      HIP_TRY(hipMemcpy(&v, t->ws.hv_cnt + 2, sizeof v, hipMemcpyDeviceToHost));
+    }
+    *value = (int64_t)v;
+    return KV_OK;
+  }
   return fail(KV_INVALID_ARGUMENT, "kv_get_stat: unknown counter %d", which);
 }
 
@@ -959,6 +1006,8 @@
   hipStream_t s = op.s;
   if ((rc = enter_op(t, s))) return rc;
   mirror_ban(t, s);
+  t->hv_banned = true;
+  if ((rc = heavy_drop(t, s))) return rc;
   unsigned c[3];
   HIP_TRY(hipMemcpyAsync(c, t->d_counters, sizeof c, hipMemcpyDeviceToHost, s));
   HIP_TRY(hipStreamSynchronize(s));
diff --git a/tfplus_amd/kv_variable/python/ops/gen_kv_variable_ops.py b/tfplus_amd/kv_variable/python/ops/gen_kv_variable_ops.py
--- a/tfplus_amd/kv_variable/python/ops/gen_kv_variable_ops.py
+++ b/tfplus_amd/kv_variable/python/ops/gen_kv_variable_ops.py
@@ -439,7 +439,7 @@
   _lib.check(_lib.lib().kv_set_fast_math(table_handle.ptr, int(bool(on))))
 
 
-KV_STAT_MIRROR_APPLIES, KV_STAT_MIRROR_EPOCHS = 0, 1
+KV_STAT_MIRROR_APPLIES, KV_STAT_MIRROR_EPOCHS, KV_STAT_HEAVY_ROUTED = 0, 1, 2
 
 
 def kv_get_stat(table_handle, which):
```

Result: slower. 7.539 billion ids/s (each id: 1 embedding lookup + 1 fused GroupAdam-V4 apply) (-4.2%).
